# ksahlin/IsoCon

Hardware: AMD Instinct MI355X
Metric: read x candidate alignments/sec (NN-graph build, 50k x 2.5kb reads) (higher is better)
Workload: dtype u64; 1 GPU; C3: 50000 synthetic CCS reads (50000 unique), ~2500 bp, 10 isoforms, seed 30001; 1-set NN graph; edges=78526, graph_digest=65944c838d76a6c9, parallelism=single GPU

## Files before the change

### isocon_amd/csrc/isocon_hip.hip

```cpp
#include <algorithm>
#include <chrono>
#include <cstdio>
#include <cstdlib>
#include <cstring>
#include <numeric>
#include <string>
#include <memory>
#include <thread>
#include <vector>

#include "common.hpp"
#include "ed_band.hpp"
#include "ed_full.hpp"
#include "qgram_mm.hpp"
#include "nn.hpp"
#include "nn_list.hpp"
#include "nn_filter.hpp"
#include "nn_finalize.hpp"
#include "nn_finalize_host.hpp"
#include "partition_host.hpp"
#include "sg.hpp"
#include "msa.hpp"
#include "msa_build.hpp"
#include "msa_batch.hpp"
#include "hw.hpp"
#include "hw_tiles.hpp"
#include "ed_lanes.hpp"
#include "ed_bytes.hpp"

namespace isocon {
thread_local std::string g_last_error;
}

using namespace isocon;

static bool variant_lookup(const char *name, std::string *value)
{
    const char *e = getenv("ISOCON_DEBUG_VARIANT");
    if (!e) return false;
    const size_t ln = strlen(name);
    for (const char *p = e; *p;) {
        const char *q = strchr(p, ',');
        const size_t len = q ? (size_t)(q - p) : strlen(p);
        if (len >= ln && strncmp(p, name, ln) == 0 && (len == ln || p[ln] == '=')) {
            if (value) *value = len > ln ? std::string(p + ln + 1, len - ln - 1) : std::string();
            return true;
        }
        p += len + (q ? 1 : 0);
    }
    return false;
}
static bool variant(const char *name) { return variant_lookup(name, nullptr); }
static const char *variant_value(const char *name)
{
    thread_local std::string ring[8];
    thread_local unsigned at = 0;
    std::string &slot = ring[at++ % 8];
    return variant_lookup(name, &slot) ? slot.c_str() : nullptr;
}

struct BoundTag {
    bool valid = false, has_order = false;
    uint64_t serial = 0;
    QMap map = {0, 0, 0, 0};
    uint32_t depth = 0;
    int32_t kcap = 0;
    unsigned long long lb_total = 0;
};
struct MsaTag { bool valid = false; uint64_t serial = 0; uint32_t n_rows = 0, n_cols = 0; };
struct MsaBatchHost {
    bool valid = false;
    uint64_t serial = 0;
    uint32_t n_parts = 0, n_rows = 0;
    std::vector<uint32_t> ncols, col_base, first_row;
    std::vector<unsigned long long> m_off;
};
struct HeldHits { uint64_t store_serial = 0; uint64_t rows = 0; };

struct ScratchPool {
    struct Slot { void *p = nullptr; size_t cap = 0; };
    Slot slots[160];
    BoundTag bound_tag;
    HeldHits held_hits;
    MsaTag msa_tag;
    MsaBatchHost msab;
    void *get(int idx, size_t bytes)
    {
        Slot &s = slots[idx];
        if (bytes == 0) bytes = 16;
        if (s.cap < bytes) {
            if (s.p) (void)hipFree(s.p);
            s.p = nullptr; s.cap = 0;
            const size_t want = bytes + bytes / 8;
            if (hipMalloc(&s.p, want) == hipSuccess) s.cap = want;
            else if (hipMalloc(&s.p, bytes) == hipSuccess) s.cap = bytes;
            else { s.p = nullptr; (void)hipGetLastError(); }
        }
        return s.p;
    }
    void release()
    {
        for (Slot &s : slots) { if (s.p) (void)hipFree(s.p); s.p = nullptr; s.cap = 0; }
        bound_tag = BoundTag();
        held_hits = HeldHits();
        msa_tag = MsaTag();
        msab = MsaBatchHost();
    }
};

enum {
    SLOT_ED_TS = 0, SLOT_ED_IDS, SLOT_ED_K, SLOT_ED_OUT, SLOT_FULL_A, SLOT_FULL_B, SLOT_FULL_K, SLOT_FULL_OUT,
    SLOT_NN_BEST, SLOT_NN_QF, SLOT_NN_TF, SLOT_NN_HITS, SLOT_NN_HITCOUNT, SLOT_NN_STATS, SLOT_NN_TS, SLOT_NN_IDS, SLOT_NN_PLANES2, SLOT_NN_PERM, SLOT_NN_IL, SLOT_NN_IL2, SLOT_NN_HITS2, SLOT_NN_HITCOUNT2, SLOT_NN_QPROF, SLOT_NN_QSUM, SLOT_NN_LB, SLOT_NN_LBROW, SLOT_NN_LBLEN, SLOT_NN_SLOTORDER, SLOT_NN_LBCHUNKS, SLOT_NN_ROWMIN, SLOT_NN_COLMIN, SLOT_NN_SEED_A, SLOT_NN_SEED_B, SLOT_NN_SEED_N, SLOT_NN_LBT, SLOT_NN_LBT_OFF, SLOT_NN_LBT_SLO, SLOT_NN_LBT_LEN, SLOT_NN_LBT_PAD, SLOT_NN_SCORE, SLOT_NN_LDEST, SLOT_NN_FIN_HITS, SLOT_NN_FIN_CNT, SLOT_NN_FIN_START, SLOT_NN_FIN_CUR, SLOT_NN_FIN_NB, SLOT_NN_FIN_LEN2, SLOT_NN_FIN_ROWPTR, SLOT_NN_FIN_COLS, SLOT_NN_FIN_FLAG, SLOT_NN_FIN_BEST, SLOT_NN_ACC_HITS, SLOT_NN_LTOT, SLOT_NN_LCHUNKS, SLOT_NN_LIST, SLOT_NN_LPA, SLOT_NN_LPB, SLOT_NN_TEXT2, SLOT_NN_LTASKS,
    SLOT_SG_PAIRS, SLOT_SG_R, SLOT_SG_TRACE, SLOT_SG_END, SLOT_SG_OPS, SLOT_SG_CNT, SLOT_SG_RES, SLOT_SG_OFF, SLOT_SG_DENSE, SLOT_SG_BOUND, SLOT_SG_AOFF, SLOT_SG_ALNA, SLOT_SG_ALNB,
    SLOT_MSA_IN, SLOT_MSA_OUT, SLOT_MSA_DEG, SLOT_MSA_COUNTS, SLOT_MSA_MAJ, SLOT_MSA_FLAGS, SLOT_MSA_TOT, SLOT_MSA_NCAND, SLOT_MSA_LEN, SLOT_MSA_OFF, SLOT_MSA_PACKED, SLOT_MSA_ROWS, SLOT_MSA_OPS, SLOT_MSA_OPTR, SLOT_MSA_LONGEST, SLOT_MSA_WIDTH, SLOT_MSA_CSLOT, SLOT_MSA_LTOT, SLOT_MSA_WIDE, SLOT_MSA_PROW, SLOT_MSA_PCOL, SLOT_MSA_PPTR, SLOT_MSA_PBYTES, SLOT_MSAB_PART, SLOT_MSAB_FIRST, SLOT_MSAB_LM, SLOT_MSAB_SBASE, SLOT_MSAB_NCOLS, SLOT_MSAB_MOFF, SLOT_MSAB_CBASE, SLOT_MSAB_CBP, SLOT_MSAB_CBC, SLOT_MSAB_CBR,
    SLOT_HW_Q, SLOT_HW_T, SLOT_HW_K, SLOT_HW_OUT, SLOT_HW_TRACE, SLOT_HW_CTR, SLOT_HW_TILEQ, SLOT_HW_LANES, SLOT_HW_PQ, SLOT_HW_KEY, SLOT_HW_HIST, SLOT_HW_CURSOR, SLOT_HW_TBASE, SLOT_HW_CLS,
    SLOT_PACK_ASCII, SLOT_PACK_OFF, SLOT_PACK_BAD, SLOT_PACK_HIST, SLOT_PACK_FLAGS, SLOT_EB_A, SLOT_EB_B, SLOT_EB_K, SLOT_EB_OUT, SLOT_EB_ROWS, SLOT_SCAN_TMP, SLOT_SCAN_SUMS,
    SLOT_COUNT
};
static_assert(SLOT_COUNT <= 160, "ScratchPool::slots too small");

static ScratchPool g_scratch;

static uint64_t g_store_serial = 0;

struct isocon_store {
    uint64_t serial = ++g_store_serial;
    DevStore dev;
    explicit isocon_store(bool private_scratch = false) : own_pool(private_scratch ? new ScratchPool() : nullptr), pool(own_pool ? *own_pool : g_scratch) {}
    std::unique_ptr<ScratchPool> own_pool;
    ScratchPool &pool;
    std::vector<int32_t> lens;
    uint64_t device_bytes = 0;
    uint64_t *d_planes = nullptr;
    char alphabet[4] = {'A', 'C', 'G', 'T'};
    bool acgt = true;
    uint8_t *d_bytes = nullptr;
    uint64_t *d_boff = nullptr;
    uint64_t bytes_base = 0;
    std::vector<uint8_t> exc;
    std::vector<uint32_t> exc_count;
    uint32_t n_exc = 0;
    bool is_exc(uint32_t i) const { return n_exc != 0 && exc[i] != 0; }
    int32_t *d_lens = nullptr;
    int32_t maxlen = 0;
};

namespace {

struct PinnedStage {
    void *p = nullptr;
    size_t cap = 0;
    void *get(size_t bytes)
    {
        if (cap < bytes) {
            if (p) (void)hipHostFree(p);
            p = nullptr; cap = 0;
            if (hipHostMalloc(&p, bytes, hipHostMallocDefault) == hipSuccess) cap = bytes;
            else { p = nullptr; (void)hipGetLastError(); }
        }
        return p;
    }
    void release() { if (p) (void)hipHostFree(p); p = nullptr; cap = 0; }
};
static PinnedStage g_stage;
static constexpr size_t kStageBytes = (size_t)32 << 20;
static constexpr uint64_t kPackWaves = (uint64_t)1 << 25;
static constexpr size_t kStageMin = (size_t)32 << 10;

static std::vector<std::pair<const char *, size_t>> g_pinned;
static bool is_pinned(const void *p, size_t bytes)
{
    for (const auto &r : g_pinned)
        if ((const char *)p >= r.first && (const char *)p + bytes <= r.first + r.second) return true;
    return false;
}

static hipError_t copy_d2h(void *dst, const void *dsrc, size_t bytes)
{
    if (bytes < kStageMin || is_pinned(dst, bytes)) return hipMemcpy(dst, dsrc, bytes, hipMemcpyDeviceToHost);
    char *st = static_cast<char *>(g_stage.get(kStageBytes));
    if (!st) return hipMemcpy(dst, dsrc, bytes, hipMemcpyDeviceToHost);
    for (size_t off = 0; off < bytes; off += kStageBytes) {
        const size_t len = std::min(kStageBytes, bytes - off);
        const hipError_t e = hipMemcpy(st, static_cast<const char *>(dsrc) + off, len, hipMemcpyDeviceToHost);
        if (e != hipSuccess) return e;
        memcpy(static_cast<char *>(dst) + off, st, len);
    }
    return hipSuccess;
}

static hipError_t copy_h2d(void *ddst, const void *src, size_t bytes)
{
    if (bytes < kStageMin || is_pinned(src, bytes)) return hipMemcpy(ddst, src, bytes, hipMemcpyHostToDevice);
    char *st = static_cast<char *>(g_stage.get(kStageBytes));
    if (!st) return hipMemcpy(ddst, src, bytes, hipMemcpyHostToDevice);
    for (size_t off = 0; off < bytes; off += kStageBytes) {
        const size_t len = std::min(kStageBytes, bytes - off);
        memcpy(st, static_cast<const char *>(src) + off, len);
        const hipError_t e = hipMemcpy(static_cast<char *>(ddst) + off, st, len, hipMemcpyHostToDevice);
        if (e != hipSuccess) return e;
    }
    return hipSuccess;
}

struct DevBuf {
    void *p = nullptr;
    ScratchPool *pool = nullptr;
    int slot = -1;
    DevBuf() {}
    DevBuf(ScratchPool *pl, int sl) : pool(pl), slot(sl) {}
    DevBuf(const DevBuf &) = delete;
    DevBuf &operator=(const DevBuf &) = delete;
    ~DevBuf() { if (p && !pool) (void)hipFree(p); }
    template <class T> T *as() { return static_cast<T *>(p); }
    int alloc(size_t bytes)
    {
        if (pool) {
            p = pool->get(slot, bytes);
            if (!p) { g_last_error = "hipMalloc(scratch slot " + std::to_string(slot) + ", " + std::to_string(bytes) + " B) failed"; return ISOCON_E_HIP; }
            return ISOCON_OK;
        }
        if (p) { (void)hipFree(p); p = nullptr; }
        ISO_HIP_CHECK(hipMalloc(&p, bytes ? bytes : 16));
        return ISOCON_OK;
    }
};

template <int SHIFT, class OUT>
static int device_exscan(ScratchPool *pl, const uint32_t *d_in, uint32_t n, OUT *d_out)
{
    DevBuf d_tmp(pl, SLOT_SCAN_TMP), d_sums(pl, SLOT_SCAN_SUMS);
    const uint32_t tiles = std::max<uint32_t>(1, (n + SCAN_TILE - 1) / SCAN_TILE);
    int rc;
    if ((rc = d_tmp.alloc((size_t)std::max<uint32_t>(n, 1) * 4)) || (rc = d_sums.alloc((size_t)tiles * 8))) return rc;
    hipLaunchKernelGGL((k_scan_tiles<SHIFT>), dim3(tiles), dim3(256), 0, 0, d_in, n, d_tmp.as<uint32_t>(), d_sums.as<unsigned long long>());
    hipLaunchKernelGGL((k_scan_finish<OUT>), dim3(tiles), dim3(256), 0, 0, d_tmp.as<uint32_t>(), n, d_sums.as<unsigned long long>(), tiles, d_out, (unsigned long long *)nullptr);
    ISO_HIP_CHECK(hipGetLastError());
    return ISOCON_OK;
}

struct EventTimer {
    hipEvent_t e0 = nullptr, e1 = nullptr, em = nullptr;
    float total = 0.f;
    float marked_total = 0.f;
    bool marked = false;
    bool ok = false;
    EventTimer() { ok = hipEventCreate(&e0) == hipSuccess && hipEventCreate(&e1) == hipSuccess && hipEventCreate(&em) == hipSuccess; }
    ~EventTimer() { if (e0) (void)hipEventDestroy(e0); if (e1) (void)hipEventDestroy(e1); if (em) (void)hipEventDestroy(em); }
    void start() { if (ok) (void)hipEventRecord(e0, 0); marked = false; }
    void mark() { if (ok) { (void)hipEventRecord(em, 0); marked = true; } }
    float stop()
    {
        float ms = 0.f;
        if (ok) {
            (void)hipEventRecord(e1, 0); (void)hipEventSynchronize(e1); (void)hipEventElapsedTime(&ms, e0, e1);
            if (marked) { float part = 0.f; (void)hipEventElapsedTime(&part, em, e1); marked_total += part; marked = false; }
        }
        total += ms;
        return ms;
    }
};

struct PackMap { uint8_t sym[4]; };

__global__ __launch_bounds__(256) void k_byte_histogram(const uint8_t *__restrict__ ascii, uint64_t total, unsigned long long *__restrict__ hist)
{
    __shared__ uint32_t h[256];
    h[threadIdx.x] = 0;
    __syncthreads();
    for (uint64_t i = (uint64_t)blockIdx.x * 256 + threadIdx.x; i < total; i += (uint64_t)gridDim.x * 256) atomicAdd(&h[ascii[i]], 1u);
    __syncthreads();
    if (h[threadIdx.x]) atomicAdd(hist + threadIdx.x, (unsigned long long)h[threadIdx.x]);
}

__global__ __launch_bounds__(256) void k_pack_planes(const uint8_t *__restrict__ ascii, const uint64_t *__restrict__ offsets, uint64_t base, uint32_t n,
                                                      uint32_t nchunks, uint64_t *__restrict__ planes, unsigned long long *__restrict__ first_bad, PackMap map,
                                                      uint32_t fold, uint64_t w0)
{
    const uint64_t w = w0 + (uint64_t)blockIdx.x * 4 + (threadIdx.x >> 6);
    if (w >= (uint64_t)nchunks * n) return;
    const uint32_t lane = threadIdx.x & 63;
    const uint32_t chunk = (uint32_t)(w / n), seq = (uint32_t)(w % n);
    const uint64_t off = offsets[seq] - base, len = offsets[seq + 1] - offsets[seq];
    const uint64_t pos = (uint64_t)chunk * 64 + lane;
    int cd = 0;
    bool bad = false;
    if (pos < len) {
        uint8_t ch = ascii[off + pos];
        if (fold && ch >= 'a' && ch <= 'z') ch = (uint8_t)(ch - 32);
        cd = ch == map.sym[0] ? 0 : ch == map.sym[1] ? 1 : ch == map.sym[2] ? 2 : ch == map.sym[3] ? 3 : -1;
        bad = cd < 0 && !fold;
    }
    const unsigned long long lo = __ballot(!bad && (cd & 1)), hi = __ballot(!bad && (cd & 2)), bm = __ballot(bad);
    if (lane == 0) {
        planes[((size_t)chunk * n + seq) * 2] = lo;
        planes[((size_t)chunk * n + seq) * 2 + 1] = hi;
        if (bm) atomicMin(first_bad, ((unsigned long long)seq << 32) | ((unsigned long long)chunk * 64 + (unsigned long long)(__ffsll((long long)bm) - 1)));
    }
}

}

extern "C" {

const char *isocon_strerror(int status)
{
    switch (status) {
    case ISOCON_OK: return "ok";
    case ISOCON_E_ARG: return "bad argument";
    case ISOCON_E_ALPHABET: return "sequence contains a symbol outside ACGT";
    case ISOCON_E_HIP: return "HIP runtime error";
    case ISOCON_E_CAPACITY: return "output buffer too small";
    case ISOCON_E_NODEVICE: return "no usable GPU";
    case ISOCON_E_UNSUPPORTED: return "unsupported request";
    default: return "unknown status";
    }
}

const char *isocon_last_error(void) { return g_last_error.c_str(); }

int isocon_device_count(void)
{
    int n = 0;
    if (hipGetDeviceCount(&n) != hipSuccess) return 0;
    return n;
}

void isocon_release_scratch(void) { g_scratch.release(); g_stage.release(); }

int isocon_init(int device_ordinal)
{
    int n = 0;
    if (hipGetDeviceCount(&n) != hipSuccess || n <= 0) { g_last_error = "hipGetDeviceCount: no device"; return ISOCON_E_NODEVICE; }
    if (device_ordinal < 0 || device_ordinal >= n) return ISOCON_E_ARG;
    ISO_HIP_CHECK(hipSetDevice(device_ordinal));
    return ISOCON_OK;
}

static int store_create_impl(const uint8_t *ascii, const uint8_t *const *seq_ptrs, const uint64_t *offsets, uint32_t n, isocon_store **out, bool private_scratch = false)
{
    *out = nullptr;
    int32_t maxlen = 0;
    for (uint32_t i = 0; i < n; ++i) {
        if (offsets[i + 1] < offsets[i] || offsets[i + 1] - offsets[i] > 0x3fffffff) return ISOCON_E_ARG;
        maxlen = std::max<int32_t>(maxlen, (int32_t)(offsets[i + 1] - offsets[i]));
    }
    const uint32_t nchunks = (uint32_t)((maxlen + 63) / 64 + 1);
    const uint32_t nn = std::max<uint32_t>(n, 1);
    std::vector<int32_t> lens(nn, 0);
    for (uint32_t i = 0; i < n; ++i) lens[i] = (int32_t)(offsets[i + 1] - offsets[i]);
    const uint64_t base = n ? offsets[0] : 0, total = n ? offsets[n] - offsets[0] : 0;
    isocon_store *st = new isocon_store(private_scratch);
    st->lens = lens;
    st->maxlen = maxlen;
    const size_t pbytes = (size_t)nchunks * nn * 2 * sizeof(uint64_t), lbytes = lens.size() * sizeof(int32_t);
    if (hipMalloc((void **)&st->d_planes, pbytes) != hipSuccess || hipMalloc((void **)&st->d_lens, lbytes) != hipSuccess) {
        g_last_error = "hipMalloc(store) failed";
        isocon_store_destroy(st);
        return ISOCON_E_HIP;
    }
    {
        DevBuf d_ascii(&g_scratch, SLOT_PACK_ASCII), d_off(&g_scratch, SLOT_PACK_OFF), d_bad(&g_scratch, SLOT_PACK_BAD);
        uint64_t pack_waves = kPackWaves;
        if (const char *e = variant_value("pack_waves")) pack_waves = std::max<uint64_t>(4, strtoull(e, nullptr, 10)) & ~(uint64_t)3;
        const unsigned long long none = ~0ull;
        int rc = ISOCON_OK;
        if ((rc = d_ascii.alloc(total ? total : 16)) || (rc = d_off.alloc((size_t)(nn + 1) * 8)) || (rc = d_bad.alloc(8))) { isocon_store_destroy(st); return rc; }
        bool up = true;
        if (total && ascii) up = copy_h2d(d_ascii.p, ascii + base, total) == hipSuccess;
        else if (total) {
            char *stg = static_cast<char *>(g_stage.get(kStageBytes));
            hipEvent_t ev[2] = {nullptr, nullptr};
            up = stg != nullptr && hipEventCreateWithFlags(&ev[0], hipEventDisableTiming) == hipSuccess && hipEventCreateWithFlags(&ev[1], hipEventDisableTiming) == hipSuccess;
            const size_t half = kStageBytes / 2;
            uint64_t done = 0;
            bool busy[2] = {false, false};
            auto gather = [&](char *dst, uint64_t b0, uint64_t b1) {
                uint32_t i = (uint32_t)(std::upper_bound(offsets, offsets + n + 1, base + b0) - offsets) - 1;
                uint64_t in_seq = base + b0 - offsets[i];
                while (b0 < b1 && i < n) {
                    const uint64_t len = offsets[i + 1] - offsets[i];
                    const size_t take = (size_t)std::min<uint64_t>(len - in_seq, b1 - b0);
                    if (take) memcpy(dst, seq_ptrs[i] + in_seq, take);
                    dst += take; b0 += take; in_seq += take;
                    if (in_seq == len) { ++i; in_seq = 0; }
                }
            };
            const unsigned hc = std::thread::hardware_concurrency();
            const unsigned n_thr = total >= ((uint64_t)8 << 20) ? std::min(4u, hc ? hc : 1u) : 1u;
            for (int h = 0; up && done < total; h ^= 1) {
                if (busy[h]) up = hipEventSynchronize(ev[h]) == hipSuccess;
                const size_t fill = (size_t)std::min<uint64_t>(half, total - done);
                if (n_thr <= 1) gather(stg + h * half, done, done + fill);
                else {
                    std::thread th[4];
                    const size_t part = (fill + n_thr - 1) / n_thr;
                    for (unsigned t = 0; t < n_thr; ++t) {
                        const size_t a = std::min(fill, t * part), b = std::min(fill, (t + 1) * part);
                        th[t] = std::thread([&, a, b, h] { if (b > a) gather(stg + h * half + a, done + a, done + b); });
                    }
                    for (unsigned t = 0; t < n_thr; ++t) th[t].join();
                }
                up = up && hipMemcpyAsync(static_cast<char *>(d_ascii.p) + done, stg + h * half, fill, hipMemcpyHostToDevice, 0) == hipSuccess &&
                     hipEventRecord(ev[h], 0) == hipSuccess;
                busy[h] = true;
                done += fill;
            }
            up = up && hipStreamSynchronize(0) == hipSuccess;
            if (ev[0]) (void)hipEventDestroy(ev[0]);
            if (ev[1]) (void)hipEventDestroy(ev[1]);
        }
        bool ok = up &&
                  (n == 0 || copy_h2d(d_off.p, offsets, (size_t)(n + 1) * 8) == hipSuccess) &&
                  hipMemcpy(d_bad.p, &none, 8, hipMemcpyHostToDevice) == hipSuccess && copy_h2d(st->d_lens, lens.data(), lbytes) == hipSuccess;
        unsigned long long bad = none;
        if (ok) {
            if (n) {
                const uint64_t waves = (uint64_t)nchunks * n;
                for (uint64_t w0 = 0; w0 < waves; w0 += pack_waves)
                    hipLaunchKernelGGL(k_pack_planes, dim3((unsigned)((std::min<uint64_t>(pack_waves, waves - w0) + 3) / 4)), dim3(256), 0, 0, d_ascii.as<uint8_t>(), d_off.as<uint64_t>(), base, n, nchunks,
                                       st->d_planes, d_bad.as<unsigned long long>(), PackMap{{'A', 'C', 'G', 'T'}}, 0u, w0);
            } else {
                ok = hipMemset(st->d_planes, 0, pbytes) == hipSuccess;
            }
            ok = ok && hipGetLastError() == hipSuccess && hipMemcpy(&bad, d_bad.p, 8, hipMemcpyDeviceToHost) == hipSuccess;
        }
        if (!ok) {
            g_last_error = "isocon_store_create: device copy / packing failed";
            (void)hipGetLastError();
            isocon_store_destroy(st);
            return ISOCON_E_HIP;
        }
        if (bad != none) {
            DevBuf d_hist(&g_scratch, SLOT_PACK_HIST);
            unsigned long long hist[256];
            bool hok = d_hist.alloc(256 * 8) == ISOCON_OK && hipMemset(d_hist.p, 0, 256 * 8) == hipSuccess;
            if (hok) {
                hipLaunchKernelGGL(k_byte_histogram, dim3(1024), dim3(256), 0, 0, d_ascii.as<uint8_t>(), (uint64_t)total, d_hist.as<unsigned long long>());
                hok = hipGetLastError() == hipSuccess && hipMemcpy(hist, d_hist.p, sizeof(hist), hipMemcpyDeviceToHost) == hipSuccess;
            }
            int distinct = 0;
            for (int c = 0; hok && c < 256; ++c) distinct += hist[c] != 0;
            if (!hok) {
                g_last_error = "isocon_store_create: symbol histogram failed";
                (void)hipGetLastError();
                isocon_store_destroy(st);
                return ISOCON_E_HIP;
            }
            if (distinct > 4) {
                DevBuf d_flags(&g_scratch, SLOT_PACK_FLAGS);
                st->exc.assign(nn, 0);
                st->exc_count.assign(nn, 0);
                bool eok = d_flags.alloc((size_t)nn * 4) == ISOCON_OK && hipMemset(d_flags.p, 0, (size_t)nn * 4) == hipSuccess &&
                           hipMalloc((void **)&st->d_bytes, total ? total : 16) == hipSuccess && hipMalloc((void **)&st->d_boff, (size_t)(nn + 1) * 8) == hipSuccess;
                if (eok) {
                    const uint64_t waves = (uint64_t)nchunks * n;
                    for (uint64_t w0 = 0; w0 < waves; w0 += pack_waves)
                    hipLaunchKernelGGL(k_pack_planes, dim3((unsigned)((std::min<uint64_t>(pack_waves, waves - w0) + 3) / 4)), dim3(256), 0, 0, d_ascii.as<uint8_t>(), d_off.as<uint64_t>(), base, n, nchunks,
                                       st->d_planes, d_bad.as<unsigned long long>(), PackMap{{'A', 'C', 'G', 'T'}}, 1u, w0);
                    for (uint64_t w0 = 0; w0 < waves; w0 += pack_waves)
                        hipLaunchKernelGGL(k_exception_flags, dim3((unsigned)((std::min<uint64_t>(pack_waves, waves - w0) + 3) / 4)), dim3(256), 0, 0, d_ascii.as<uint8_t>(), d_off.as<uint64_t>(), base, n,
                                           nchunks, d_flags.as<uint32_t>(), (uint32_t)'A' | ((uint32_t)'C' << 8) | ((uint32_t)'G' << 16) | ((uint32_t)'T' << 24), w0);
                    eok = hipGetLastError() == hipSuccess && hipMemcpy(st->exc_count.data(), d_flags.p, (size_t)n * 4, hipMemcpyDeviceToHost) == hipSuccess &&
                          hipMemcpy(st->d_bytes, d_ascii.p, total, hipMemcpyDeviceToDevice) == hipSuccess &&
                          hipMemcpy(st->d_boff, d_off.p, (size_t)(n + 1) * 8, hipMemcpyDeviceToDevice) == hipSuccess;
                }
                if (!eok) {
                    g_last_error = "isocon_store_create: keeping the bytes of a set with more than four symbols failed";
                    (void)hipGetLastError();
                    isocon_store_destroy(st);
                    return ISOCON_E_HIP;
                }
                st->bytes_base = base;
                for (uint32_t i = 0; i < n; ++i) { st->exc[i] = st->exc_count[i] != 0; st->n_exc += st->exc[i]; }
                st->acgt = false;
                st->device_bytes += total + (size_t)(nn + 1) * 8;
            } else {
            PackMap map{{0, 0, 0, 0}};
            bool used[4] = {false, false, false, false};
            const char acgt_sym[4] = {'A', 'C', 'G', 'T'};
            for (int k = 0; k < 4; ++k) if (hist[(uint8_t)acgt_sym[k]]) { map.sym[k] = (uint8_t)acgt_sym[k]; used[k] = true; }
            for (int c = 0; c < 256; ++c) {
                if (!hist[c] || c == 'A' || c == 'C' || c == 'G' || c == 'T') continue;
                for (int k = 0; k < 4; ++k) if (!used[k]) { map.sym[k] = (uint8_t)c; used[k] = true; break; }
            }
            for (int k = 0; k < 4; ++k) if (!used[k]) { for (int c = 1; c < 256; ++c) if (!hist[c] && c != map.sym[0] && c != map.sym[1] && c != map.sym[2] && c != map.sym[3]) { map.sym[k] = (uint8_t)c; break; } }
            bool rok = hipMemcpy(d_bad.p, &none, 8, hipMemcpyHostToDevice) == hipSuccess;
            if (rok) {
                const uint64_t waves = (uint64_t)nchunks * n;
                for (uint64_t w0 = 0; w0 < waves; w0 += pack_waves)
                    hipLaunchKernelGGL(k_pack_planes, dim3((unsigned)((std::min<uint64_t>(pack_waves, waves - w0) + 3) / 4)), dim3(256), 0, 0, d_ascii.as<uint8_t>(), d_off.as<uint64_t>(), base, n, nchunks,
                                       st->d_planes, d_bad.as<unsigned long long>(), map, 0u, w0);
                rok = hipGetLastError() == hipSuccess && hipMemcpy(&bad, d_bad.p, 8, hipMemcpyDeviceToHost) == hipSuccess && bad == none;
            }
            if (!rok) {
                g_last_error = "isocon_store_create: packing under the set's own alphabet failed";
                (void)hipGetLastError();
                isocon_store_destroy(st);
                return ISOCON_E_HIP;
            }
            for (int k = 0; k < 4; ++k) st->alphabet[k] = (char)map.sym[k];
            st->acgt = false;
            }
        }
    }
    st->device_bytes += pbytes + lbytes;
    st->dev.planes = st->d_planes;
    st->dev.il = nullptr;
    st->dev.lens = st->d_lens;
    st->dev.n = n;
    st->dev.nchunks = nchunks;
    st->lens.resize(n);
    *out = st;
    return ISOCON_OK;
}

int isocon_store_create(const uint8_t *ascii, const uint64_t *offsets, uint32_t n, isocon_store **out)
{
    if (!out || (!ascii && n) || !offsets) return ISOCON_E_ARG;
    return store_create_impl(ascii, nullptr, offsets, n, out);
}

int isocon_store_create_ptrs(const uint8_t *const *seq_ptrs, const uint64_t *seq_lens, uint32_t n, isocon_store **out)
{
    if (!out || (n && (!seq_ptrs || !seq_lens))) return ISOCON_E_ARG;
    std::vector<uint64_t> offsets((size_t)n + 1, 0);
    for (uint32_t i = 0; i < n; ++i) {
        if (seq_lens[i] && !seq_ptrs[i]) return ISOCON_E_ARG;
        offsets[i + 1] = offsets[i] + seq_lens[i];
    }
    return store_create_impl(nullptr, seq_ptrs, offsets.data(), n, out);
}

int isocon_store_create_ptrs_ex(const uint8_t *const *seq_ptrs, const uint64_t *seq_lens, uint32_t n, uint32_t flags, isocon_store **out)
{
    if (!out || (n && (!seq_ptrs || !seq_lens)) || (flags & ~(uint32_t)ISOCON_STORE_PRIVATE_SCRATCH)) return ISOCON_E_ARG;
    std::vector<uint64_t> offsets((size_t)n + 1, 0);
    for (uint32_t i = 0; i < n; ++i) {
        if (seq_lens[i] && !seq_ptrs[i]) return ISOCON_E_ARG;
        offsets[i + 1] = offsets[i] + seq_lens[i];
    }
    return store_create_impl(nullptr, seq_ptrs, offsets.data(), n, out, (flags & ISOCON_STORE_PRIVATE_SCRATCH) != 0);
}

void *isocon_host_alloc(uint64_t bytes)
{
    void *p = nullptr;
    if (hipHostMalloc(&p, bytes ? bytes : 16, hipHostMallocDefault) != hipSuccess) { (void)hipGetLastError(); return nullptr; }
    g_pinned.emplace_back((const char *)p, (size_t)(bytes ? bytes : 16));
    return p;
}

void isocon_host_free(void *p)
{
    if (!p) return;
    for (size_t i = 0; i < g_pinned.size(); ++i)
        if (g_pinned[i].first == (const char *)p) { g_pinned.erase(g_pinned.begin() + (long)i); break; }
    (void)hipHostFree(p);
}

void isocon_store_destroy(isocon_store *s)
{
    if (!s) return;
    if (s->d_planes) (void)hipFree(s->d_planes);
    if (s->d_lens) (void)hipFree(s->d_lens);
    if (s->d_bytes) (void)hipFree(s->d_bytes);
    if (s->d_boff) (void)hipFree(s->d_boff);
    if (s->own_pool) s->own_pool->release();
    delete s;
}

uint32_t isocon_store_size(const isocon_store *s) { return s ? s->dev.n : 0; }
uint64_t isocon_store_device_bytes(const isocon_store *s) { return s ? s->device_bytes : 0; }

}

namespace {

template <int W>
int launch_band_tiles(isocon_store *st, const DevStore &S, const std::vector<uint32_t> &tile_shared, const std::vector<uint32_t> &lane_ids,
                      const std::vector<int32_t> &lane_k, std::vector<int32_t> &out, EventTimer &tm)
{
    const size_t nt = tile_shared.size();
    out.assign(nt * 64, -1);
    if (!nt) return ISOCON_OK;
    DevBuf d_ts(&st->pool, SLOT_ED_TS), d_ids(&st->pool, SLOT_ED_IDS), d_k(&st->pool, SLOT_ED_K), d_out(&st->pool, SLOT_ED_OUT);
    int rc;
    if ((rc = d_ts.alloc(nt * 4)) || (rc = d_ids.alloc(nt * 64 * 4)) || (rc = d_k.alloc(nt * 64 * 4)) || (rc = d_out.alloc(nt * 64 * 4))) return rc;
    ISO_HIP_CHECK(copy_h2d(d_ts.p, tile_shared.data(), nt * 4));
    ISO_HIP_CHECK(copy_h2d(d_ids.p, lane_ids.data(), nt * 64 * 4));
    ISO_HIP_CHECK(copy_h2d(d_k.p, lane_k.data(), nt * 64 * 4));
    tm.start();
    hipLaunchKernelGGL(k_ed_band_tiles<W>, dim3((unsigned)((nt + 3) / 4)), dim3(256), 0, 0, S, d_ts.as<uint32_t>(),
                       d_ids.as<uint32_t>(), d_k.as<int32_t>(), d_out.as<int32_t>(), (uint32_t)nt);
    ISO_HIP_CHECK(hipGetLastError());
    tm.stop();
    ISO_HIP_CHECK(copy_d2h(out.data(), d_out.p, nt * 64 * 4));
    return ISOCON_OK;
}

int run_band_stage(int W, isocon_store *st, const DevStore &S, const std::vector<uint32_t> &ts, const std::vector<uint32_t> &ids,
                   const std::vector<int32_t> &ks, std::vector<int32_t> &out, EventTimer &tm)
{
    switch (W) {
    case 1: return launch_band_tiles<1>(st, S, ts, ids, ks, out, tm);
    case 2: return launch_band_tiles<2>(st, S, ts, ids, ks, out, tm);
    case 4: return launch_band_tiles<4>(st, S, ts, ids, ks, out, tm);
    case 8: return launch_band_tiles<8>(st, S, ts, ids, ks, out, tm);
    default: return ISOCON_E_ARG;
    }
}

int run_full(isocon_store *st, const std::vector<uint32_t> &a, const std::vector<uint32_t> &b,
             const std::vector<int32_t> &k, std::vector<int32_t> &out, EventTimer &tm)
{
    const size_t np = a.size();
    out.assign(np, -1);
    if (!np) return ISOCON_OK;
    DevBuf d_a(&st->pool, SLOT_FULL_A), d_b(&st->pool, SLOT_FULL_B), d_k(&st->pool, SLOT_FULL_K), d_out(&st->pool, SLOT_FULL_OUT);
    int rc;
    if ((rc = d_a.alloc(np * 4)) || (rc = d_b.alloc(np * 4)) || (rc = d_k.alloc(np * 4)) || (rc = d_out.alloc(np * 4))) return rc;
    ISO_HIP_CHECK(copy_h2d(d_a.p, a.data(), np * 4));
    ISO_HIP_CHECK(copy_h2d(d_b.p, b.data(), np * 4));
    ISO_HIP_CHECK(copy_h2d(d_k.p, k.data(), np * 4));
    bool multipass = false;
    int32_t maxtext = 0;
    for (size_t p = 0; p < np; ++p) {
        const int32_t la = st->lens[a[p]], lb = st->lens[b[p]];
        if (std::min(la, lb) > 4096) multipass = true;
        maxtext = std::max(maxtext, std::max(la, lb));
    }
    const size_t lds = multipass ? (size_t)((maxtext + 15) & ~15) : 0;
    if (lds > 160 * 1024) { g_last_error = "sequence longer than 163840 bases in the un-banded kernel"; return ISOCON_E_UNSUPPORTED; }
    if (lds > 64 * 1024)
        ISO_HIP_CHECK(hipFuncSetAttribute((const void *)k_ed_full, hipFuncAttributeMaxDynamicSharedMemorySize, (int)lds));
    tm.start();
    hipLaunchKernelGGL(k_ed_full, dim3((unsigned)np), dim3(64), lds, 0, st->dev, d_a.as<uint32_t>(), d_b.as<uint32_t>(),
                       d_k.as<int32_t>(), d_out.as<int32_t>(), (uint32_t)np);
    ISO_HIP_CHECK(hipGetLastError());
    tm.stop();
    ISO_HIP_CHECK(copy_d2h(out.data(), d_out.p, np * 4));
    return ISOCON_OK;
}

int run_bytes(isocon_store *st, const std::vector<uint32_t> &a, const std::vector<uint32_t> &b, const std::vector<int32_t> &k, std::vector<int32_t> &out, EventTimer &tm)
{
    const size_t np = a.size();
    out.assign(np, -1);
    if (!np) return ISOCON_OK;
    if (!st->d_bytes) { g_last_error = "internal: byte-wise distances on a store that kept no bytes"; return ISOCON_E_HIP; }
    if (st->maxlen >= (int32_t)EB_INF - 1) { g_last_error = "byte-wise distances: sequences of 8 388 606 bases and more are not supported"; return ISOCON_E_UNSUPPORTED; }
    const uint32_t row_stride = (uint32_t)st->maxlen + 130u;
    size_t waves = std::min<size_t>(np, 8192);
    while (waves > 256 && waves * row_stride * 4 > ((size_t)2 << 30)) waves /= 2;
    DevBuf d_a(&st->pool, SLOT_EB_A), d_b(&st->pool, SLOT_EB_B), d_k(&st->pool, SLOT_EB_K), d_out(&st->pool, SLOT_EB_OUT), d_rows(&st->pool, SLOT_EB_ROWS);
    int rc;
    if ((rc = d_a.alloc(np * 4)) || (rc = d_b.alloc(np * 4)) || (rc = d_k.alloc(np * 4)) || (rc = d_out.alloc(np * 4)) || (rc = d_rows.alloc(waves * row_stride * 4))) return rc;
    ISO_HIP_CHECK(copy_h2d(d_a.p, a.data(), np * 4));
    ISO_HIP_CHECK(copy_h2d(d_b.p, b.data(), np * 4));
    ISO_HIP_CHECK(copy_h2d(d_k.p, k.data(), np * 4));
    tm.start();
    hipLaunchKernelGGL(k_ed_bytes, dim3((unsigned)waves), dim3(64), 0, 0, ByteStore{st->d_bytes, st->d_boff, st->bytes_base, st->d_lens}, d_a.as<uint32_t>(), d_b.as<uint32_t>(),
                       d_k.as<int32_t>(), (unsigned long long)np, d_rows.as<uint32_t>(), row_stride, d_out.as<int32_t>());
    ISO_HIP_CHECK(hipGetLastError());
    tm.stop();
    ISO_HIP_CHECK(copy_d2h(out.data(), d_out.p, np * 4));
    return ISOCON_OK;
}

}

namespace isocon {

int ed_pairs_impl(isocon_store *st, const uint32_t *a, const uint32_t *b, const int32_t *k, uint64_t n_pairs,
                  int32_t *out_ed, float *kernel_ms, uint64_t *full_pairs, bool images)
{
    EventTimer tm;
    const uint32_t n = st->dev.n;
    for (uint64_t p = 0; p < n_pairs; ++p)
        if (a[p] >= n || b[p] >= n) return ISOCON_E_ARG;
    bool swap_roles = false;
    {
        std::vector<uint8_t> seen_a(n, 0), seen_b(n, 0);
        size_t da = 0, db = 0;
        for (uint64_t p = 0; p < n_pairs; ++p) {
            if (!seen_a[a[p]]) { seen_a[a[p]] = 1; ++da; }
            if (!seen_b[b[p]]) { seen_b[b[p]] = 1; ++db; }
        }
        swap_roles = db < da;
    }
    std::vector<uint64_t> pending;
    pending.reserve(n_pairs);
    if (st->n_exc && !images) {
        std::vector<uint64_t> xp;
        for (uint64_t p = 0; p < n_pairs; ++p) (st->exc[a[p]] || st->exc[b[p]] ? xp : pending).push_back(p);
        if (!xp.empty()) {
            std::vector<uint32_t> xa(xp.size()), xb(xp.size());
            std::vector<int32_t> xk(xp.size()), res;
            for (size_t i = 0; i < xp.size(); ++i) { xa[i] = a[xp[i]]; xb[i] = b[xp[i]]; xk[i] = k ? k[xp[i]] : -1; }
            int rc = run_bytes(st, xa, xb, xk, res, tm);
            if (rc) return rc;
            for (size_t i = 0; i < xp.size(); ++i) out_ed[xp[i]] = res[i];
        }
    } else {
        pending.resize(n_pairs);
        std::iota(pending.begin(), pending.end(), 0);
    }
    static const int stages[4] = {1, 2, 4, 8};
    for (int si = 0; si < 4 && !pending.empty(); ++si) {
        const int W = stages[si];
        const int32_t kcap = 64 * W - 1;
        auto sh = [&](uint64_t p) { return swap_roles ? b[p] : a[p]; };
        auto ln = [&](uint64_t p) { return swap_roles ? a[p] : b[p]; };
        std::sort(pending.begin(), pending.end(), [&](uint64_t x, uint64_t y) {
            if (sh(x) != sh(y)) return sh(x) < sh(y);
            const int32_t lx = st->lens[ln(x)], ly = st->lens[ln(y)];
            if (lx != ly) return lx < ly;
            return x < y;
        });
        std::vector<uint64_t> todo = pending, next;
        if (W == 1) {
            const char *e = variant_value("ed_lanes");
            const size_t min_group = e ? (atoi(e) ? (size_t)-1 : 0) : 16;
            std::vector<uint64_t> lanes_p, tiles_p;
            for (size_t i = 0; i < todo.size();) {
                size_t j = i;
                while (j < todo.size() && sh(todo[j]) == sh(todo[i])) ++j;
                std::vector<uint64_t> &dst = (j - i) < min_group ? lanes_p : tiles_p;
                dst.insert(dst.end(), todo.begin() + i, todo.begin() + j);
                i = j;
            }
            if (!lanes_p.empty()) {
                const size_t np = lanes_p.size();
                std::vector<uint32_t> la(np), lb2(np);
                std::vector<int32_t> lk(np), res(np, -1);
                for (size_t i = 0; i < np; ++i) {
                    const uint64_t p = lanes_p[i];
                    la[i] = a[p]; lb2[i] = b[p];
                    const int32_t kr = k ? k[p] : -1;
                    lk[i] = kr < 0 ? kcap : std::min(kr, kcap);
                }
                DevBuf d_a(&st->pool, SLOT_ED_TS), d_b(&st->pool, SLOT_ED_IDS), d_k(&st->pool, SLOT_ED_K), d_out(&st->pool, SLOT_ED_OUT);
                int rc;
                if ((rc = d_a.alloc(np * 4)) || (rc = d_b.alloc(np * 4)) || (rc = d_k.alloc(np * 4)) || (rc = d_out.alloc(np * 4))) return rc;
                ISO_HIP_CHECK(copy_h2d(d_a.p, la.data(), np * 4));
                ISO_HIP_CHECK(copy_h2d(d_b.p, lb2.data(), np * 4));
                ISO_HIP_CHECK(copy_h2d(d_k.p, lk.data(), np * 4));
                NNParams none;
                memset(&none, 0, sizeof(none));
                tm.start();
                hipLaunchKernelGGL(k_ed_lanes<false>, dim3((unsigned)((np + 255) / 256)), dim3(256), 0, 0, st->dev, none, d_a.as<uint32_t>(), d_b.as<uint32_t>(),
                                   d_k.as<int32_t>(), (uint64_t)np, d_out.as<int32_t>());
                ISO_HIP_CHECK(hipGetLastError());
                tm.stop();
                ISO_HIP_CHECK(copy_d2h(res.data(), d_out.p, np * 4));
                for (size_t i = 0; i < np; ++i) {
                    const uint64_t p = lanes_p[i];
                    const int32_t kr = k ? k[p] : -1;
                    if (res[i] >= 0) out_ed[p] = res[i];
                    else if (kr >= 0 && kr <= kcap) out_ed[p] = -1;
                    else next.push_back(p);
                }
            }
            todo.swap(tiles_p);
        }
        for (int round = 0; round < 2 && !todo.empty(); ++round) {
            std::vector<uint32_t> ts, ids;
            std::vector<int32_t> ks;
            std::vector<uint64_t> slot_pair;
            size_t i = 0;
            while (i < todo.size()) {
                size_t j = i;
                const uint32_t s0 = sh(todo[i]);
                const size_t lim = round == 0 ? 64 : 1;
                while (j < todo.size() && j - i < lim && sh(todo[j]) == s0) ++j;
                ts.push_back(s0);
                for (size_t l = 0; l < 64; ++l) {
                    if (i + l < j) {
                        const uint64_t p = todo[i + l];
                        ids.push_back(ln(p));
                        const int32_t kr = k ? k[p] : -1;
                        ks.push_back(kr < 0 ? kcap : std::min(kr, kcap));
                        slot_pair.push_back(p);
                    } else {
                        ids.push_back(0xffffffffu);
                        ks.push_back(-1);
                        slot_pair.push_back(~(uint64_t)0);
                    }
                }
                i = j;
            }
            std::vector<int32_t> res;
            int rc = run_band_stage(W, st, st->dev, ts, ids, ks, res, tm);
            if (rc) return rc;
            std::vector<uint64_t> retry;
            for (size_t sidx = 0; sidx < slot_pair.size(); ++sidx) {
                const uint64_t p = slot_pair[sidx];
                if (p == ~(uint64_t)0) continue;
                const int32_t r = res[sidx];
                const int32_t kr = k ? k[p] : -1;
                if (r >= 0) out_ed[p] = r;
                else if (r == -2) retry.push_back(p);
                else if (kr >= 0 && kr <= kcap) out_ed[p] = -1;
                else next.push_back(p);
            }
            todo.swap(retry);
        }
        if (!todo.empty()) { g_last_error = "internal: single-lane tile undetermined"; return ISOCON_E_HIP; }
        pending.swap(next);
    }
    if (full_pairs) *full_pairs = pending.size();
    if (!pending.empty()) {
        std::vector<uint32_t> fa, fb;
        std::vector<int32_t> fk, res;
        for (uint64_t p : pending) { fa.push_back(a[p]); fb.push_back(b[p]); fk.push_back(k ? k[p] : -1); }
        int rc = run_full(st, fa, fb, fk, res, tm);
        if (rc) return rc;
        for (size_t i = 0; i < pending.size(); ++i) out_ed[pending[i]] = res[i];
    }
    if (kernel_ms) *kernel_ms = tm.total;
    return ISOCON_OK;
}

}

__global__ __launch_bounds__(256) void k_store_digest(const uint64_t *__restrict__ planes, size_t n_words, const int32_t *__restrict__ lens, uint32_t n,
                                                      unsigned long long *__restrict__ out)
{
    unsigned long long acc = 0;
    const size_t stride = (size_t)gridDim.x * blockDim.x;
    for (size_t i = (size_t)blockIdx.x * blockDim.x + threadIdx.x; i < n_words + n; i += stride) {
        unsigned long long v = i < n_words ? planes[i] : (unsigned long long)(uint32_t)lens[i - n_words];
        v ^= (unsigned long long)i * 0xD6E8FEB86659FD93ull;
        v ^= v >> 32; v *= 0x9E3779B97F4A7C15ull; v ^= v >> 29; v *= 0xBF58476D1CE4E5B9ull; v ^= v >> 32;
        acc += v;
    }
    for (int o = 32; o > 0; o >>= 1) acc += __shfl_xor(acc, o, 64);
    if ((threadIdx.x & 63) == 0 && acc) atomicAdd(out, acc);
}

extern "C" int isocon_store_digest(const isocon_store *s, uint64_t *out)
{
    if (!s || !out) return ISOCON_E_ARG;
    DevBuf d_acc;
    int rc;
    if ((rc = d_acc.alloc(8))) return rc;
    ISO_HIP_CHECK(hipMemset(d_acc.p, 0, 8));
    const size_t n_words = (size_t)s->dev.nchunks * std::max<uint32_t>(s->dev.n, 1) * 2;
    hipLaunchKernelGGL(k_store_digest, dim3(1024), dim3(256), 0, 0, s->d_planes, n_words, s->d_lens, s->dev.n, d_acc.as<unsigned long long>());
    ISO_HIP_CHECK(hipGetLastError());
    ISO_HIP_CHECK(hipMemcpy(out, d_acc.p, 8, hipMemcpyDeviceToHost));
    return ISOCON_OK;
}

extern "C" int isocon_ed_pairs(isocon_store *s, const uint32_t *a, const uint32_t *b, const int32_t *k, uint64_t n_pairs,
                               int32_t *out_ed, float *kernel_ms)
{
    if (!s || (n_pairs && (!a || !b || !out_ed))) return ISOCON_E_ARG;
    if (kernel_ms) *kernel_ms = 0.f;
    if (!n_pairs) return ISOCON_OK;
    return ed_pairs_impl(s, a, b, k, n_pairs, out_ed, kernel_ms, nullptr, false);
}

extern "C" int isocon_qgram_params(int32_t *out)
{
    if (out) { out[0] = QG_Q; out[1] = QG_B0; out[2] = QG_B1; out[3] = QG_CAP; }
    return QM_K;
}

namespace isocon {
int qgram_bounds_for_pairs(isocon_store *s, const uint32_t *a, const uint32_t *b, uint64_t n_pairs, int32_t *out_bound, float *kernel_ms)
{
    const uint32_t n = s->dev.n;
    const uint32_t n_pad = std::max<uint32_t>(QM_TILE, ((n + QM_TILE - 1) / QM_TILE) * QM_TILE);
    DevBuf d_prof(&s->pool, SLOT_NN_QPROF), d_sum(&s->pool, SLOT_NN_QSUM), d_a(&s->pool, SLOT_ED_TS), d_b(&s->pool, SLOT_ED_IDS), d_out(&s->pool, SLOT_ED_OUT);
    int rc;
    if ((rc = d_prof.alloc((size_t)n_pad * (QM_K / 2))) || (rc = d_sum.alloc((size_t)n * 4)) || (rc = d_a.alloc(n_pairs * 4)) || (rc = d_b.alloc(n_pairs * 4)) ||
        (rc = d_out.alloc(n_pairs * 4)))
        return rc;
    s->pool.bound_tag.valid = false;
    ISO_HIP_CHECK(copy_h2d(d_a.p, a, n_pairs * 4));
    ISO_HIP_CHECK(copy_h2d(d_b.p, b, n_pairs * 4));
    EventTimer tm;
    tm.start();
    hipLaunchKernelGGL(k_qgram_profile4, dim3((n + QP_SEQS - 1) / QP_SEQS), dim3(256), 0, 0, s->dev, d_prof.as<uint8_t>(), d_sum.as<uint32_t>(), n_pad);
    ISO_HIP_CHECK(hipGetLastError());
    for (uint64_t at = 0; at < n_pairs; at += (uint64_t)1 << 24) {
        const uint64_t cnt = std::min<uint64_t>((uint64_t)1 << 24, n_pairs - at);
        hipLaunchKernelGGL(k_qgram_lb_pairs, dim3((unsigned)((cnt + 3) / 4)), dim3(256), 0, 0, d_prof.as<uint8_t>(), d_sum.as<uint32_t>(), n_pad, d_a.as<uint32_t>() + at,
                           d_b.as<uint32_t>() + at, cnt, d_out.as<int32_t>() + at);
        ISO_HIP_CHECK(hipGetLastError());
    }
    const float ms = tm.stop();
    if (kernel_ms) *kernel_ms = ms;
    ISO_HIP_CHECK(copy_d2h(out_bound, d_out.p, n_pairs * 4));
    return ISOCON_OK;
}
}

extern "C" int isocon_qgram_bound_pairs(isocon_store *s, const uint32_t *a, const uint32_t *b, uint64_t n_pairs, int32_t *out_bound)
{
    if (!s || (n_pairs && (!a || !b || !out_bound))) return ISOCON_E_ARG;
    if (!n_pairs) return ISOCON_OK;
    if (s->n_exc) { g_last_error = "q-gram bounds are defined on the 2-bit planes: the set holds more than four distinct symbols"; return ISOCON_E_ALPHABET; }
    const uint32_t n = s->dev.n;
    for (uint64_t i = 0; i < n_pairs; ++i)
        if (a[i] >= n || b[i] >= n) { g_last_error = "pair index out of range"; return ISOCON_E_ARG; }
    return qgram_bounds_for_pairs(s, a, b, n_pairs, out_bound, nullptr);
}

extern "C" int isocon_block_bound_pairs(isocon_store *s, const uint32_t *owner, const uint32_t *partner, uint64_t n_pairs, int32_t probe_stride, int32_t *out_count)
{
    if (probe_stride != 4 && probe_stride != 2) return ISOCON_E_ARG;
    if (!s || (n_pairs && (!owner || !partner || !out_count))) return ISOCON_E_ARG;
    if (!n_pairs) return ISOCON_OK;
    if (s->n_exc) { g_last_error = "block bounds are defined on the 2-bit planes: the set holds more than four distinct symbols"; return ISOCON_E_ALPHABET; }
    const uint32_t n = s->dev.n;
    if (n_pairs >= ((uint64_t)1 << 31)) return ISOCON_E_ARG;
    for (uint64_t i = 0; i < n_pairs; ++i)
        if (owner[i] >= n || partner[i] >= n) { g_last_error = "pair index out of range"; return ISOCON_E_ARG; }
    const uint32_t stride = nnf_text2_stride(s->maxlen);
    DevBuf d_text(&s->pool, SLOT_NN_TEXT2), d_a(&s->pool, SLOT_ED_TS), d_b(&s->pool, SLOT_ED_IDS), d_out(&s->pool, SLOT_ED_OUT);
    int rc;
    if ((rc = d_text.alloc((size_t)n * stride * 4)) || (rc = d_a.alloc(n_pairs * 4)) || (rc = d_b.alloc(n_pairs * 4)) || (rc = d_out.alloc(n_pairs * 4))) return rc;
    ISO_HIP_CHECK(copy_h2d(d_a.p, owner, n_pairs * 4));
    ISO_HIP_CHECK(copy_h2d(d_b.p, partner, n_pairs * 4));
    hipLaunchKernelGGL(k_build_text2, dim3(n), dim3(256), 0, 0, s->dev, d_text.as<uint32_t>(), stride);
    hipLaunchKernelGGL(k_nn_block_count_pairs, dim3((unsigned)n_pairs), dim3(256), 0, 0, d_text.as<uint32_t>(), stride, s->dev.lens, d_a.as<uint32_t>(), d_b.as<uint32_t>(), d_out.as<int32_t>(), probe_stride);
    ISO_HIP_CHECK(hipGetLastError());
    ISO_HIP_CHECK(copy_d2h(out_count, d_out.p, n_pairs * 4));
    return ISOCON_OK;
}

#include "nn_context.inc"
#include "nn_bounds.inc"
#include "nn_lists.inc"
#include "nn_main.inc"
#include "nn_wide.inc"
#include "nn_images.inc"
#include "nn_entry.inc"
#include "sg_host.inc"
#include "msa_host.inc"
#include "hw_host.inc"

extern "C" int isocon_partition_ids(uint32_t n, const int32_t *degree, uint64_t n_edges, const uint32_t *edge_a, const uint32_t *edge_b,
                                    const uint32_t *rank, int32_t nbr_tiebreak, uint32_t *out_centre, int64_t *out_weight,
                                    uint64_t *out_member_ptr, uint32_t *out_members, uint32_t *n_parts)
{
    if (!out_member_ptr || !n_parts || (n && (!degree || !rank || !out_centre || !out_weight || !out_members)) || (n_edges && (!edge_a || !edge_b))) return ISOCON_E_ARG;
    return partition_ids_impl(n, degree, n_edges, edge_a, edge_b, rank, nbr_tiebreak, out_centre, out_weight, out_member_ptr, out_members, n_parts);
}
```

### isocon_amd/csrc/nn_bounds.inc

```

namespace {

int NNContext::build_bounds(const QMap &Q, int32_t kcap, NNParams &P, bool want_seeds)
{
    const uint32_t q_begin = Q.begin, q_end = Q.end;
    P.lb = nullptr;
    P.lb_row = nullptr;
    P.slot_order = nullptr;
    if (variant("nn_no_qgram") || n < 2 || n >= (1u << 30) || q_begin >= q_end) return ISOCON_OK;
    if (!want_seeds && st->pool.bound_tag.valid && st->pool.bound_tag.serial == st->serial && st->pool.bound_tag.map.same(Q) &&
        st->pool.bound_tag.depth == depth && st->pool.bound_tag.kcap == kcap) {
        P.lb = static_cast<const uint8_t *>(st->pool.slots[SLOT_NN_LB].p);
        P.lb_row = static_cast<const unsigned long long *>(st->pool.slots[SLOT_NN_LBROW].p);
        if (st->pool.bound_tag.has_order && use_slot_order(Q.count())) P.slot_order = static_cast<const uint32_t *>(st->pool.slots[SLOT_NN_SLOTORDER].p);
        lb_total = st->pool.bound_tag.lb_total;
        return ISOCON_OK;
    }
    st->pool.bound_tag.valid = false;
    const uint32_t nq = Q.count();
    const std::vector<int32_t> &lens = st->lens;
    const uint32_t n_pad = std::max<uint32_t>(QM_TILE, ((n + QM_TILE - 1) / QM_TILE) * QM_TILE);
    const size_t prof_bytes = (size_t)n_pad * (QM_K / 2);
    d_qprof.pool = d_qsum.pool = &st->pool;
    d_qprof.slot = SLOT_NN_QPROF; d_qsum.slot = SLOT_NN_QSUM;
    HostClock bclk;
    {
        size_t free_b = 0, total_b = 0;
        if (hipMemGetInfo(&free_b, &total_b) != hipSuccess || prof_bytes > free_b / 2 + st->pool.slots[SLOT_NN_QPROF].cap) return ISOCON_OK;
        if (d_qprof.alloc(prof_bytes) || d_qsum.alloc((size_t)n * 4)) return ISOCON_OK;
    }
    bclk.lap("bounds: memory check + profile buffers");
    tm.start();
    hipLaunchKernelGGL(k_qgram_profile4, dim3((n + QP_SEQS - 1) / QP_SEQS), dim3(256), 0, 0, st->dev, d_qprof.as<uint8_t>(), d_qsum.as<uint32_t>(), n_pad);
    ISO_HIP_CHECK(hipGetLastError());
    struct StopTimer { NNContext &c; bool armed = true; ~StopTimer() { if (armed) c.stats.bound_kernel_ms += c.tm.stop(); } } stop_timer{*this};
    std::vector<unsigned long long> &off = lb_off_host;
    std::vector<uint32_t> &rlen = lb_len_host;
    off.assign(nq, 0);
    rlen.assign(nq, 0);
    unsigned long long total = 0, sum_rlen = 0;
    uint64_t hi = 0;
    const uint32_t nrb = (nq + QM_TILE - 1) / QM_TILE;
    std::vector<uint64_t> rb_lo(nrb, ~(uint64_t)0), rb_hi(nrb, 0);
    for (uint32_t s = 0; s < nq; ++s) {
        const uint64_t q = Q.entry(s);
        if (hi < q + 1) hi = q + 1;
        while (hi < n && lens[hi] - lens[q] <= kcap) ++hi;
        uint64_t len = hi - q - 1;
        if (len > depth) len = depth;
        const uint64_t pal = (q + 1) & ~(uint64_t)15;
        off[s] = total + (q + 1 - pal);
        rlen[s] = (uint32_t)len;
        sum_rlen += len;
        if (len) {
            total += ((q + 1 + len + 15) & ~(uint64_t)15) - pal;
            rb_lo[s / QM_TILE] = std::min<uint64_t>(rb_lo[s / QM_TILE], q + 1);
            rb_hi[s / QM_TILE] = std::max<uint64_t>(rb_hi[s / QM_TILE], q + len);
        }
    }
    if (total == 0) return ISOCON_OK;
    bclk.lap("bounds: profile launch + rows (host)");
    const unsigned long long totalT = sum_rlen + 30ull * n;
    bclk.lap("bounds: transposed rows (host)");
    size_t free_b = 0, total_b = 0;
    const size_t need = (size_t)total + (size_t)totalT + prof_bytes + (size_t)n * 24 + (size_t)nq * 12;
    if (hipMemGetInfo(&free_b, &total_b) != hipSuccess || need > free_b / 2 + st->pool.slots[SLOT_NN_LB].cap + st->pool.slots[SLOT_NN_QPROF].cap) return ISOCON_OK;
    bclk.lap("bounds: memory check 2");
    std::vector<uint2> tiles;
    for (uint32_t g = 0; g * 4 < nrb; ++g) {
        uint64_t jmin = ~(uint64_t)0, jmax = 0;
        bool any = false;
        for (uint32_t I = g * 4; I < std::min(nrb, g * 4 + 4); ++I)
            if (rb_lo[I] != ~(uint64_t)0) { any = true; jmin = std::min(jmin, rb_lo[I] / QM_TILE); jmax = std::max(jmax, rb_hi[I] / QM_TILE); }
        if (!any) continue;
        for (uint64_t j0 = jmin; j0 <= jmax; j0 += 8)
            for (uint32_t ri = 0; ri < 4; ++ri)
                for (uint32_t cj = 0; cj < 8; ++cj) {
                    const uint32_t I = g * 4 + ri;
                    const uint64_t J = j0 + cj;
                    const bool have = I < nrb && rb_lo[I] != ~(uint64_t)0 && J >= rb_lo[I] / QM_TILE && J <= rb_hi[I] / QM_TILE;
                    tiles.push_back(have ? make_uint2(I, (uint32_t)J) : make_uint2(0xffffffffu, 0xffffffffu));
                }
    }
    while (tiles.size() % 256) tiles.push_back(make_uint2(0xffffffffu, 0xffffffffu));
    if (tiles.size() > 0x7fffffffull) return ISOCON_OK;
    bclk.lap("bounds: tile table (host)");
    d_lb.pool = d_lbrow.pool = d_lblen.pool = &st->pool;
    d_lb.slot = SLOT_NN_LB; d_lbrow.slot = SLOT_NN_LBROW; d_lblen.slot = SLOT_NN_LBLEN;
    int rc;
    if ((rc = d_lb.alloc((size_t)total)) ||
        (rc = d_lbrow.alloc((size_t)nq * 8)) || (rc = d_lblen.alloc((size_t)nq * 4)))
        return ISOCON_OK;
    d_lbt.pool = d_offT.pool = d_sloT.pool = d_lenT.pool = d_score.pool = &st->pool;
    d_lbt.slot = SLOT_NN_LBT; d_offT.slot = SLOT_NN_LBT_OFF; d_sloT.slot = SLOT_NN_LBT_SLO; d_lenT.slot = SLOT_NN_LBT_LEN; d_score.slot = SLOT_NN_SCORE;
    DevBuf d_padT(&st->pool, SLOT_NN_LBT_PAD);
    if (d_lbt.alloc((size_t)totalT + 16) || d_offT.alloc(((size_t)n + 1) * 8) || d_sloT.alloc((size_t)n * 4) || d_lenT.alloc((size_t)n * 4) || d_score.alloc((size_t)n * 4) ||
        d_padT.alloc((size_t)n * 4))
        return ISOCON_OK;
    ISO_HIP_CHECK(hipMemsetAsync(d_score.p, 0, (size_t)n * 4, 0));
    d_chunks.pool = &st->pool;
    d_chunks.slot = SLOT_NN_LBCHUNKS;
    if (d_chunks.alloc(tiles.size() * sizeof(uint2))) return ISOCON_OK;
    ISO_HIP_CHECK(copy_h2d(d_chunks.p, tiles.data(), tiles.size() * sizeof(uint2)));
    ISO_HIP_CHECK(copy_h2d(d_lbrow.p, off.data(), (size_t)nq * 8));
    ISO_HIP_CHECK(copy_h2d(d_lblen.p, rlen.data(), (size_t)nq * 4));
    hipLaunchKernelGGL(k_lbt_rows, dim3((n + 255) / 256), dim3(256), 0, 0, Q, nq, d_lblen.as<uint32_t>(), n, d_sloT.as<uint32_t>(), d_lenT.as<uint32_t>(), d_padT.as<uint32_t>());
    if ((rc = device_exscan<0, unsigned long long>(&st->pool, d_padT.as<uint32_t>(), n, d_offT.as<unsigned long long>()))) return ISOCON_OK;
    hipLaunchKernelGGL(k_lbt_offsets, dim3((n + 255) / 256), dim3(256), 0, 0, n, d_sloT.as<uint32_t>(), d_offT.as<unsigned long long>());
    ISO_HIP_CHECK(hipGetLastError());
    bclk.lap("bounds: alloc + uploads");
    if (use_slot_order(nq)) {
        std::vector<uint32_t> order(nq);
        std::iota(order.begin(), order.end(), 0u);
        std::stable_sort(order.begin(), order.end(), [&](uint32_t x, uint32_t y) { return rlen[x] > rlen[y]; });
        d_order.pool = &st->pool;
        d_order.slot = SLOT_NN_SLOTORDER;
        if (d_order.alloc((size_t)nq * 4)) return ISOCON_OK;
        ISO_HIP_CHECK(copy_h2d(d_order.p, order.data(), (size_t)nq * 4));
    }
    unsigned long long *rowmin = nullptr, *colmin = nullptr;
    if (want_seeds) {
        d_rowmin.pool = d_colmin.pool = d_seed_a.pool = d_seed_b.pool = &st->pool;
        d_rowmin.slot = SLOT_NN_ROWMIN; d_colmin.slot = SLOT_NN_COLMIN; d_seed_a.slot = SLOT_NN_SEED_A; d_seed_b.slot = SLOT_NN_SEED_B;
        if (!(d_rowmin.alloc((size_t)nq * 8 * QM_SEEDS) || d_colmin.alloc((size_t)n_pad * 8 * QM_SEEDS) || d_seed_a.alloc((size_t)n * 8 * QM_SEEDS) || d_seed_b.alloc((size_t)n * 8 * QM_SEEDS))) {
            ISO_HIP_CHECK(hipMemsetAsync(d_rowmin.p, 0xff, (size_t)nq * 8 * QM_SEEDS, 0));
            ISO_HIP_CHECK(hipMemsetAsync(d_colmin.p, 0xff, (size_t)n_pad * 8 * QM_SEEDS, 0));
            rowmin = d_rowmin.as<unsigned long long>();
            colmin = d_colmin.as<unsigned long long>();
        }
    }
    bclk.lap("bounds: slot order + seed buffers");
    static bool lds_attr_set = false;
    if (!lds_attr_set) {
        ISO_HIP_CHECK(hipFuncSetAttribute((const void *)k_qgram_mm, hipFuncAttributeMaxDynamicSharedMemorySize, (int)QM_LDS_BYTES));
        lds_attr_set = true;
    }
    tm.mark();
    hipLaunchKernelGGL(k_qgram_mm, dim3((unsigned)tiles.size()), dim3(512), QM_LDS_BYTES, 0, d_qprof.as<uint8_t>(), d_qsum.as<uint32_t>(), n, n_pad,
                       d_chunks.as<uint2>(), d_lbrow.as<unsigned long long>(), d_lblen.as<uint32_t>(), d_lb.as<uint8_t>(), Q, nq,
                       d_qf.as<uint8_t>(), d_tf.as<uint8_t>(), rowmin, colmin, d_offT.as<unsigned long long>(), d_sloT.as<uint32_t>(), d_lenT.as<uint32_t>(),
                       d_lbt.as<uint8_t>(), d_score.as<uint32_t>());
    ISO_HIP_CHECK(hipGetLastError());
    stop_timer.armed = false;
    {
        const float before = tm.marked_total;
        stats.bound_kernel_ms += tm.stop();
        stats.mm_kernel_ms += tm.marked_total - before;
        tm.marked_total = before;
    }
    bclk.lap("bounds: k_qgram_mm (wait)");
#ifdef ISOCON_QM_TIMELINE
    {
        const size_t nt = std::min<size_t>(tiles.size(), 16384);
        std::vector<unsigned long long> tl(nt * 8);
        ISO_HIP_CHECK(hipMemcpyFromSymbol(tl.data(), HIP_SYMBOL(g_qm_timeline), nt * 64));
        double sum[5] = {0, 0, 0, 0, 0};
        unsigned long long t_min = ~0ull, t_max = 0;
        size_t cnt = 0;
        for (size_t b = 0; b < nt; ++b) {
            if (tiles[b].x == 0xffffffffu) continue;
            const unsigned long long *t = tl.data() + b * 8;
            for (int k = 0; k < 5; ++k) sum[k] += (double)(t[k + 1] - t[k]);
            t_min = std::min(t_min, t[0]); t_max = std::max(t_max, t[5]);
            ++cnt;
        }
        fprintf(stderr, "[qm timeline] %zu tiles: prologue %.2f us, K loop %.2f us, E1 %.2f us, E2 %.2f us, E3 %.2f us per tile; first start to last end %.3f ms\n", cnt,
                sum[0] / cnt / 100.0, sum[1] / cnt / 100.0, sum[2] / cnt / 100.0, sum[3] / cnt / 100.0, sum[4] / cnt / 100.0, (double)(t_max - t_min) / 1e5);
    }
#endif
    for (const uint2 &t : tiles) stats.bound_tiles += t.x != 0xffffffffu;
    P.lb = d_lb.as<uint8_t>();
    P.lb_row = d_lbrow.as<unsigned long long>();
    if (use_slot_order(nq)) P.slot_order = d_order.as<uint32_t>();
    seeds_ready = rowmin != nullptr;
    seed_nq = nq;
    lb_total = total;
    st->pool.bound_tag.valid = true;
    st->pool.bound_tag.lb_total = total;
    st->pool.bound_tag.has_order = use_slot_order(nq);
    st->pool.bound_tag.serial = st->serial;
    st->pool.bound_tag.map = Q; st->pool.bound_tag.depth = depth; st->pool.bound_tag.kcap = kcap;
    return ISOCON_OK;
}

int NNContext::run_bound_seeds(const QMap &Q)
{
    if (!seeds_ready) return ISOCON_OK;
    tm.start();
    const uint64_t np = (uint64_t)2 * QM_SEEDS * n;
    const uint32_t ranks = std::max<uint32_t>(1u, Q.stride >> Q.block_log2);
    uint32_t col_classes = QM_SEEDS;
    while (col_classes > 1 && col_classes * ranks > (uint32_t)QM_SEEDS) col_classes >>= 1;
    if (const char *e = variant_value("nn_seed_classes")) { const int v = atoi(e); if (v == 1 || v == 2 || v == QM_SEEDS) col_classes = (uint32_t)v; }
    DevBuf d_seed_n(&st->pool, SLOT_NN_SEED_N);
    int rc;
    if ((rc = d_seed_n.alloc(8))) return rc;
    ISO_HIP_CHECK(hipMemsetAsync(d_seed_n.p, 0, 8, 0));
    ISO_HIP_CHECK(hipMemsetAsync(d_seed_a.p, 0xff, (size_t)np * 4, 0));
    ISO_HIP_CHECK(hipMemsetAsync(d_seed_b.p, 0xff, (size_t)np * 4, 0));
    hipLaunchKernelGGL(k_qgram_seed_pairs, dim3((n + 255) / 256), dim3(256), 0, 0, d_rowmin.as<unsigned long long>(), d_colmin.as<unsigned long long>(),
                       n, Q, seed_nq, col_classes, d_seed_a.as<uint32_t>(), d_seed_b.as<uint32_t>(), d_seed_n.as<unsigned long long>());
    ISO_HIP_CHECK(hipGetLastError());
    hipLaunchKernelGGL(k_ed_lanes<true>, dim3((unsigned)((np + 255) / 256)), dim3(256), 0, 0, st->dev, params(63), d_seed_a.as<uint32_t>(), d_seed_b.as<uint32_t>(),
                       (const int32_t *)nullptr, np, (int32_t *)nullptr);
    ISO_HIP_CHECK(hipGetLastError());
    stats.seed_kernel_ms += tm.stop();
    return ISOCON_OK;
}

}
```

### isocon_amd/csrc/nn_context.inc

```

namespace {

struct HostClock {
    std::chrono::steady_clock::time_point t0 = std::chrono::steady_clock::now();
    const bool on = getenv("ISOCON_DEBUG") != nullptr;
    void lap(const char *what)
    {
        if (!on) return;
        const auto t1 = std::chrono::steady_clock::now();
        fprintf(stderr, "[isocon] %-28s %8.2f ms\n", what, std::chrono::duration<double, std::milli>(t1 - t0).count());
        t0 = t1;
    }
};

struct NNContext {
    isocon_store *st = nullptr;
    uint32_t n = 0;
    std::vector<uint8_t> qflag, tflag;
    bool two_set = false;
    std::vector<uint8_t> wide_mask;
    int32_t min_d = 1;
    uint32_t depth = 0x7fffffffu;
    DevBuf d_best, d_qf, d_tf, d_hits, d_hit_count, d_stats;
    DevBuf d_text;
    uint32_t text_stride = 0;
    bool text_ready = false;
    DevBuf d_qprof, d_qsum, d_lb, d_lbrow, d_lblen;
    DevBuf d_chunks;
    DevBuf d_lbt, d_offT, d_sloT, d_lenT, d_score;
    DevBuf d_order;
    DevBuf d_rowmin, d_colmin, d_seed_a, d_seed_b;
    uint64_t hits_cap = 0;
    std::vector<int32_t> best;
    std::vector<int32_t> hits;
    isocon_nn_stats stats;
    EventTimer tm;

    bool ensure_text()
    {
        if (text_ready) return true;
        text_stride = (uint32_t)NN_TEXT_PAD_FRONT + (uint32_t)((st->maxlen + 7) / 8) + (uint32_t)NN_TEXT_PAD_BACK;
        size_t free_b = 0, total_b = 0;
        if (hipMemGetInfo(&free_b, &total_b) != hipSuccess || (size_t)n * text_stride * 4 > free_b / 2) return false;
        d_text.pool = &st->pool;
        d_text.slot = SLOT_NN_IL;
        if (d_text.alloc((size_t)std::max<uint32_t>(n, 1) * text_stride * 4) != ISOCON_OK) return false;
        hipLaunchKernelGGL(k_build_nibble_text, dim3(std::max<uint32_t>(n, 1)), dim3(256), 0, 0, st->dev, d_text.as<uint32_t>(), text_stride);
        if (hipGetLastError() != hipSuccess) return false;
        text_ready = true;
        return true;
    }
    DevBuf d_text2;
    uint32_t text2_stride = 0;
    bool text2_ready = false;
    bool ensure_text2()
    {
        if (text2_ready) return true;
        text2_stride = nnf_text2_stride(st->maxlen);
        size_t free_b = 0, total_b = 0;
        if (hipMemGetInfo(&free_b, &total_b) != hipSuccess || (size_t)n * text2_stride * 4 > free_b / 2 + st->pool.slots[SLOT_NN_TEXT2].cap) return false;
        d_text2.pool = &st->pool;
        d_text2.slot = SLOT_NN_TEXT2;
        if (d_text2.alloc((size_t)std::max<uint32_t>(n, 1) * text2_stride * 4) != ISOCON_OK) return false;
        hipLaunchKernelGGL(k_build_text2, dim3(std::max<uint32_t>(n, 1)), dim3(256), 0, 0, st->dev, d_text2.as<uint32_t>(), text2_stride);
        if (hipGetLastError() != hipSuccess) return false;
        text2_ready = true;
        return true;
    }
    static bool use_slot_order(uint32_t nq)
    {
        if (const char *e = variant_value("nn_order")) return atoi(e) != 0;
        return nq <= 16384;
    }
    int build_bounds(const QMap &Q, int32_t kcap, NNParams &P, bool want_seeds = false);
    std::vector<unsigned long long> lb_off_host;
    std::vector<uint32_t> lb_len_host;
    unsigned long long lb_total = 0;
    bool seeds_ready = false;
    uint32_t seed_nq = 0;
    int run_bound_seeds(const QMap &Q);
    DevBuf d_ltot, d_lchunks, d_list, d_lpa, d_lpb, d_lmeta, d_ltasks;
    struct ListPlan {
        bool listed = false;
        unsigned long long n_chunks = 0, n_chunks_narrow = 0, n_small = 0;
        unsigned long long conv_a = 0, conv_b = 0, conv_pairs = 0;
        NNChunk *a = nullptr, *b = nullptr, *sorted_a = nullptr, *sorted_b = nullptr;
    };
    int plan_lists(const QMap &Q, uint32_t nq, const NNParams &PR, ListPlan &L);
    NNParams params(int32_t kcap)
    {
        NNParams P;
        P.best = d_best.as<int32_t>();
        P.qflag = d_qf.as<uint8_t>();
        P.tflag = d_tf.as<uint8_t>();
        P.hits = d_hits.as<int32_t>();
        P.hit_count = d_hit_count.as<unsigned long long>();
        P.stats = d_stats.as<unsigned long long>();
        P.hits_cap = hits_cap;
        P.kcap = kcap;
        P.min_d = image_pass ? 0 : min_d;
        P.depth = depth;
        P.fixed = fixed ? 1 : 0;
        P.q_list = nullptr;
        P.own = QMap{0u, n, 1u, 0u};
        P.lb = nullptr;
        P.lb_row = nullptr;
        P.slot_order = nullptr;
        P.wg_base = 0;
        P.chunks = nullptr;
        P.list = nullptr;
        return P;
    }

    int upload_best() { ISO_HIP_CHECK(copy_h2d(d_best.p, best.data(), (size_t)n * 4)); return ISOCON_OK; }
    int download_best() { ISO_HIP_CHECK(copy_d2h(best.data(), d_best.p, (size_t)n * 4)); return ISOCON_OK; }
    int reset_counters()
    {
        ISO_HIP_CHECK(hipMemset(d_hit_count.p, 0, 8));
        ISO_HIP_CHECK(hipMemset(d_stats.p, 0, 2 * (NN_COUNTER_SLOTS * 4 + 1) * 8));
        return ISOCON_OK;
    }
    bool keep_dev = false;
    const int32_t *dev_hits = nullptr;
    uint64_t dev_hit_count = 0;
    int collect(std::vector<int32_t> &out, uint64_t *needed, bool filter = false, bool to_device = false)
    {
        unsigned long long cnt = 0;
        ISO_HIP_CHECK(hipMemcpy(&cnt, d_hit_count.p, 8, hipMemcpyDeviceToHost));
        unsigned long long sc2[2][NN_COUNTER_SLOTS * 4 + 1];
        ISO_HIP_CHECK(hipMemcpy(sc2, d_stats.p, sizeof(sc2), hipMemcpyDeviceToHost));
        for (int blk = 0; blk < 2; ++blk) {
            const unsigned long long *sc = sc2[blk];
            stats.pairs_prefiltered += sc[NN_COUNTER_SLOTS * 4];
            for (int i = 0; i < NN_COUNTER_SLOTS; ++i) {
                stats.pairs_evaluated += sc[i * 4 + 0];
                stats.cells_columns += sc[i * 4 + 1];
                stats.tiles += sc[i * 4 + 2];
                stats.live_columns += sc[i * 4 + 3];
                if (blk == 1) stats.narrow_columns += sc[i * 4 + 1];
            }
        }
        if (needed) *needed = cnt;
        if (cnt > hits_cap) return ISOCON_E_CAPACITY;
        stats.hits += cnt;
        const void *src = d_hits.p;
        if (filter && cnt > 4096 && dev_hit_count == 0) {
            DevBuf d_h2(&st->pool, SLOT_NN_HITS2), d_c2(&st->pool, SLOT_NN_HITCOUNT2);
            int rc;
            if ((rc = d_h2.alloc((size_t)cnt * 12)) || (rc = d_c2.alloc(8))) return rc;
            ISO_HIP_CHECK(hipMemset(d_c2.p, 0, 8));
            const unsigned blocks = (unsigned)std::min<unsigned long long>((cnt + 255) / 256, 4096);
            hipLaunchKernelGGL(k_filter_hits, dim3(blocks), dim3(256), 0, 0, d_hits.as<int32_t>(), cnt, d_best.as<int32_t>(), d_h2.as<int32_t>(),
                               d_c2.as<unsigned long long>());
            ISO_HIP_CHECK(hipGetLastError());
            ISO_HIP_CHECK(hipMemcpy(&cnt, d_c2.p, 8, hipMemcpyDeviceToHost));
            src = d_h2.p;
        }
        if (to_device) {
            dev_hits = static_cast<const int32_t *>(src);
            dev_hit_count = cnt;
            return ISOCON_OK;
        }
        const size_t base = out.size();
        out.resize(base + (size_t)cnt * 3);
        if (cnt) ISO_HIP_CHECK(copy_d2h(out.data() + base, src, (size_t)cnt * 12));
        return ISOCON_OK;
    }
    int pull_dev_hits()
    {
        if (dev_hit_count) {
            const size_t base = hits.size();
            hits.resize(base + (size_t)dev_hit_count * 3);
            ISO_HIP_CHECK(copy_d2h(hits.data() + base, dev_hits, (size_t)dev_hit_count * 12));
        }
        dev_hits = nullptr;
        dev_hit_count = 0;
        return ISOCON_OK;
    }
    bool is_exc(uint32_t q) const { return st->n_exc != 0 && st->exc[q] != 0; }
    bool mask_exc = true;
    bool image_pass = false;
    bool fixed = false;
    bool dev_excluded(uint32_t q) const { return mask_exc && is_exc(q); }
    bool flags_dirty = false;
    int upload_flags()
    {
        if (!n) return ISOCON_OK;
        if (!st->n_exc || !mask_exc) {
            ISO_HIP_CHECK(copy_h2d(d_qf.p, qflag.data(), n));
            ISO_HIP_CHECK(copy_h2d(d_tf.p, tflag.data(), n));
            return ISOCON_OK;
        }
        std::vector<uint8_t> q2(qflag), t2(tflag);
        for (uint32_t i = 0; i < n; ++i)
            if (st->exc[i]) q2[i] = t2[i] = 0;
        ISO_HIP_CHECK(copy_h2d(d_qf.p, q2.data(), n));
        ISO_HIP_CHECK(copy_h2d(d_tf.p, t2.data(), n));
        return ISOCON_OK;
    }
    bool admissible(uint32_t x, uint32_t y) const { return qflag[x] && tflag[y]; }
    void apply(uint32_t s, uint32_t p, int32_t d)
    {
        if (d < min_d) return;
        const int32_t ls = st->lens[s], lp = st->lens[p];
        if (admissible(s, p) && d <= ls && d <= best[s]) { if (!fixed) best[s] = d; hits.push_back((int32_t)s); hits.push_back((int32_t)p); hits.push_back(d); }
        if (admissible(p, s) && d <= lp && d <= best[p]) { if (!fixed) best[p] = d; hits.push_back((int32_t)p); hits.push_back((int32_t)s); hits.push_back(d); }
    }
};

template <int W>
int launch_nn_tiles(NNContext &C, const std::vector<uint32_t> &ts, const std::vector<uint32_t> &ids, int32_t kcap, float *ms_out)
{
    const size_t nt = ts.size();
    if (!nt) return ISOCON_OK;
    DevBuf d_ts(&C.st->pool, SLOT_NN_TS), d_ids(&C.st->pool, SLOT_NN_IDS);
    int rc;
    if ((rc = d_ts.alloc(nt * 4)) || (rc = d_ids.alloc(nt * 64 * 4))) return rc;
    ISO_HIP_CHECK(copy_h2d(d_ts.p, ts.data(), nt * 4));
    ISO_HIP_CHECK(copy_h2d(d_ids.p, ids.data(), nt * 64 * 4));
    C.tm.start();
    hipLaunchKernelGGL(k_nn_tiles<W>, dim3((unsigned)((nt + 3) / 4)), dim3(256), 0, 0, C.st->dev, C.params(kcap),
                       d_ts.as<uint32_t>(), d_ids.as<uint32_t>(), (uint32_t)nt);
    ISO_HIP_CHECK(hipGetLastError());
    const float ms = C.tm.stop();
    if (ms_out) *ms_out += ms;
    return ISOCON_OK;
}

int run_nn_tiles(int W, NNContext &C, const std::vector<uint32_t> &ts, const std::vector<uint32_t> &ids, float *ms_out)
{
    switch (W) {
    case 1: return launch_nn_tiles<1>(C, ts, ids, 63, ms_out);
    case 2: return launch_nn_tiles<2>(C, ts, ids, 127, ms_out);
    case 4: return launch_nn_tiles<4>(C, ts, ids, 255, ms_out);
    case 8: return launch_nn_tiles<8>(C, ts, ids, 511, ms_out);
    default: return ISOCON_E_ARG;
    }
}

void push_tiles(std::vector<uint32_t> &ts, std::vector<uint32_t> &ids, uint32_t shared, const std::vector<uint32_t> &lanes)
{
    for (size_t i = 0; i < lanes.size(); i += 64) {
        ts.push_back(shared);
        for (size_t l = 0; l < 64; ++l) ids.push_back(i + l < lanes.size() ? lanes[i + l] : 0xffffffffu);
    }
}

void length_window(const std::vector<int32_t> &lens, uint32_t x, int32_t w, uint32_t &lo, uint32_t &hi)
{
    const int32_t L = lens[x];
    lo = (uint32_t)(std::lower_bound(lens.begin(), lens.end(), L - w) - lens.begin());
    hi = (uint32_t)(std::upper_bound(lens.begin(), lens.end(), L + w) - lens.begin());
}

int nn_setup(NNContext &C, isocon_store *s, const uint8_t *is_converged, const uint8_t *is_target, uint64_t depth,
             const int32_t *best_in)
{
    C.st = s;
    C.n = s->dev.n;
    C.d_best.pool = C.d_qf.pool = C.d_tf.pool = C.d_hits.pool = C.d_hit_count.pool = C.d_stats.pool = &s->pool;
    C.d_best.slot = SLOT_NN_BEST; C.d_qf.slot = SLOT_NN_QF; C.d_tf.slot = SLOT_NN_TF; C.d_hits.slot = SLOT_NN_HITS;
    C.d_hit_count.slot = SLOT_NN_HITCOUNT; C.d_stats.slot = SLOT_NN_STATS;
    const uint32_t n = C.n;
    for (uint32_t i = 1; i < n; ++i)
        if (s->lens[i] < s->lens[i - 1]) { g_last_error = "nearest-neighbour entry points need a length-sorted store"; return ISOCON_E_ARG; }
    C.two_set = is_target != nullptr;
    C.min_d = C.two_set ? 0 : 1;
    C.qflag.assign(n, 0);
    C.tflag.assign(n, 0);
    uint64_t n_targets = 0;
    for (uint32_t i = 0; i < n; ++i) {
        if (C.two_set) { C.tflag[i] = is_target[i] ? 1 : 0; C.qflag[i] = is_target[i] ? 0 : 1; n_targets += C.tflag[i]; }
        else { C.tflag[i] = 1; C.qflag[i] = (is_converged && is_converged[i]) ? 0 : 1; }
    }
    if (C.two_set) {
        if (depth < n_targets) { g_last_error = "2-set search with neighbor_search_depth < number of targets is not supported"; return ISOCON_E_UNSUPPORTED; }
        C.depth = 0x7fffffffu;
    } else {
        if (depth == 0) { g_last_error = "neighbor_search_depth must be >= 1"; return ISOCON_E_ARG; }
        C.depth = depth > 0x7fffffffull ? 0x7fffffffu : (uint32_t)depth;
    }
    HostClock clk;
    C.best.assign(std::max<uint32_t>(n, 1), NN_INF);
    if (best_in) std::copy(best_in, best_in + n, C.best.begin());
    clk.lap("setup: host arrays");
    memset(&C.stats, 0, sizeof(C.stats));
    C.hits_cap = ((uint64_t)1 << 20) + (uint64_t)n * 48;
    if (const char *e = variant_value("hits_cap")) C.hits_cap = std::max<uint64_t>(16, strtoull(e, nullptr, 10));
    int rc;
    if ((rc = C.d_best.alloc((size_t)std::max<uint32_t>(n, 1) * 4)) || (rc = C.d_qf.alloc(std::max<uint32_t>(n, 1))) ||
        (rc = C.d_tf.alloc(std::max<uint32_t>(n, 1))) || (rc = C.d_hits.alloc(C.hits_cap * 12)) || (rc = C.d_hit_count.alloc(8)) ||
        (rc = C.d_stats.alloc(2 * (NN_COUNTER_SLOTS * 4 + 1) * 8)))
        return rc;
    clk.lap("setup: pool");
    if ((rc = C.upload_flags())) return rc;
    clk.lap("setup: role flags");
    return ISOCON_OK;
}

bool qmap_args_ok(uint32_t q_stride, uint32_t q_block) { return q_stride != 0 && q_block != 0 && (q_block & (q_block - 1)) == 0 && q_block <= q_stride; }
QMap qmap_of(uint32_t q_begin, uint32_t q_end, uint32_t q_stride, uint32_t q_block)
{
    uint32_t lg = 0;
    while ((1u << lg) < q_block) ++lg;
    return QMap{q_begin, q_end, q_stride, lg};
}

}
```

### isocon_amd/csrc/nn_entry.inc

```

namespace {

int nn_phase_a(NNContext &C, const QMap &Q, bool allow_regroup = false, bool do_seed = true, bool do_main = true, bool seeded_before = false)
{
    if (!C.st->n_exc || !do_main) return nn_phase_a_planes(C, Q, allow_regroup, do_seed, do_main, seeded_before);
    return nn_phase_a_images(C, Q, allow_regroup, do_seed, seeded_before);
}

int nn_phase_b(NNContext &C, const QMap &Q)
{
    return C.st->n_exc ? nn_phase_b_images(C, Q) : nn_phase_b_planes(C, Q);
}


int nn_finalize_device_core(ScratchPool *pl, uint32_t n, const int32_t *d_best, const int32_t *best_host, const int32_t *d_hits, uint64_t n_hits,
                            int32_t *out_best, uint64_t *out_row_ptr, uint32_t *out_cols, uint64_t cols_cap, uint64_t *n_cols_needed)
{
    DevBuf d_cnt(pl, SLOT_NN_FIN_CNT), d_start(pl, SLOT_NN_FIN_START), d_cur(pl, SLOT_NN_FIN_CUR), d_nb(pl, SLOT_NN_FIN_NB),
        d_len2(pl, SLOT_NN_FIN_LEN2), d_rowptr(pl, SLOT_NN_FIN_ROWPTR), d_cols(pl, SLOT_NN_FIN_COLS), d_flag(pl, SLOT_NN_FIN_FLAG);
    int rc;
    if ((rc = d_cnt.alloc((size_t)n * 4)) || (rc = d_start.alloc(((size_t)n + 1) * 8)) || (rc = d_cur.alloc((size_t)n * 4)) ||
        (rc = d_nb.alloc((size_t)n_hits * 4 + 16)) || (rc = d_len2.alloc((size_t)n * 4)) || (rc = d_rowptr.alloc(((size_t)n + 1) * 8)) ||
        (rc = d_cols.alloc((size_t)n_hits * 4 + 16)) || (rc = d_flag.alloc(4)))
        return rc;
    ISO_HIP_CHECK(hipMemsetAsync(d_cnt.p, 0, (size_t)n * 4, 0));
    ISO_HIP_CHECK(hipMemsetAsync(d_cur.p, 0, (size_t)n * 4, 0));
    ISO_HIP_CHECK(hipMemsetAsync(d_flag.p, 0, 4, 0));
    const unsigned hb = (unsigned)std::max<uint64_t>(1, (n_hits + 255) / 256), nb_ = (n + 255) / 256;
    hipLaunchKernelGGL(k_fin_count, dim3(hb), dim3(256), 0, 0, d_hits, (unsigned long long)n_hits, d_best, n, d_cnt.as<uint32_t>());
    if ((rc = device_exscan<0, unsigned long long>(pl, d_cnt.as<uint32_t>(), n, d_start.as<unsigned long long>()))) return rc;
    hipLaunchKernelGGL(k_fin_scatter, dim3(hb), dim3(256), 0, 0, d_hits, (unsigned long long)n_hits, d_best, n,
                       d_start.as<unsigned long long>(), d_cur.as<uint32_t>(), d_nb.as<uint32_t>());
    hipLaunchKernelGGL(k_fin_rows, dim3(nb_), dim3(256), 0, 0, n, d_start.as<unsigned long long>(), d_nb.as<uint32_t>(), d_len2.as<uint32_t>(), d_flag.as<uint32_t>());
    if ((rc = device_exscan<0, unsigned long long>(pl, d_len2.as<uint32_t>(), n, d_rowptr.as<unsigned long long>()))) return rc;
    hipLaunchKernelGGL(k_fin_gather, dim3(nb_), dim3(256), 0, 0, n, d_start.as<unsigned long long>(), d_nb.as<uint32_t>(), d_rowptr.as<unsigned long long>(), d_cols.as<uint32_t>());
    ISO_HIP_CHECK(hipGetLastError());
    uint32_t flag = 0;
    ISO_HIP_CHECK(hipMemcpy(&flag, d_flag.p, 4, hipMemcpyDeviceToHost));
    if (flag) return ISOCON_E_UNSUPPORTED;
    static_assert(sizeof(unsigned long long) == sizeof(uint64_t), "row pointers travel as they are");
    ISO_HIP_CHECK(copy_d2h(out_row_ptr, d_rowptr.p, ((size_t)n + 1) * 8));
    const uint64_t total = out_row_ptr[n];
    if (n_cols_needed) *n_cols_needed = total;
    if (total > cols_cap) return ISOCON_E_CAPACITY;
    if (total) ISO_HIP_CHECK(copy_d2h(out_cols, d_cols.p, (size_t)total * 4));
    for (uint32_t i = 0; i < n; ++i) out_best[i] = out_row_ptr[i + 1] > out_row_ptr[i] ? best_host[i] : -1;
    return ISOCON_OK;
}

int nn_finalize_device(isocon_store *st, uint32_t n, const int32_t *best, const int32_t *hits, uint64_t n_hits, int32_t *out_best,
                       uint64_t *out_row_ptr, uint32_t *out_cols, uint64_t cols_cap, uint64_t *n_cols_needed)
{
    ScratchPool *pl = &st->pool;
    DevBuf d_hits(pl, SLOT_NN_FIN_HITS), d_best(pl, SLOT_NN_FIN_BEST);
    int rc;
    if ((rc = d_hits.alloc((size_t)n_hits * 12)) || (rc = d_best.alloc((size_t)n * 4))) return rc;
    ISO_HIP_CHECK(copy_h2d(d_hits.p, hits, (size_t)n_hits * 12));
    ISO_HIP_CHECK(copy_h2d(d_best.p, best, (size_t)n * 4));
    return nn_finalize_device_core(pl, n, d_best.as<int32_t>(), best, d_hits.as<int32_t>(), n_hits, out_best, out_row_ptr, out_cols, cols_cap, n_cols_needed);
}


}

extern "C" int isocon_nn_partial(isocon_store *s, const uint8_t *is_converged, const uint8_t *is_target, uint64_t depth,
                                 uint32_t q_begin, uint32_t q_end, uint32_t q_stride, uint32_t q_block, int32_t phase, int32_t *best_inout,
                                 int32_t *out_hits, uint64_t hits_cap, uint64_t *n_hits, isocon_nn_stats *stats, const uint8_t *wide_queries)
{
    if (!s || !best_inout || !n_hits || (hits_cap && !out_hits) || phase < 0 || phase > 3 || !qmap_args_ok(q_stride, q_block)) return ISOCON_E_ARG;
    const uint32_t n = s->dev.n;
    if (q_end > n) q_end = n;
    const QMap Q = qmap_of(q_begin, q_end, q_stride, q_block);
    NNContext C;
    int rc = nn_setup(C, s, is_converged, is_target, depth, best_inout);
    if (rc) return rc;
    if (phase == 2 && wide_queries) C.wide_mask.assign(wide_queries, wide_queries + n);
    rc = phase == 2 ? nn_phase_b(C, Q) : nn_phase_a(C, Q, false, phase == 0 || phase == 3, phase == 1 || phase == 3, phase == 1);
    if (rc) return rc;
    C.stats.kernel_ms = C.tm.total; C.stats.narrow_kernel_ms = C.tm.marked_total;
    if (stats) *stats = C.stats;
    std::copy(C.best.begin(), C.best.begin() + n, best_inout);
    *n_hits = C.hits.size() / 3;
    if (*n_hits > hits_cap) return ISOCON_E_CAPACITY;
    if (!C.hits.empty()) memcpy(out_hits, C.hits.data(), C.hits.size() * 4);
    return ISOCON_OK;
}

extern "C" int isocon_nn_finalize(uint32_t n, const int32_t *best, const int32_t *hits, uint64_t n_hits,
                                  int32_t *out_best, uint64_t *out_row_ptr, uint32_t *out_cols, uint64_t cols_cap,
                                  uint64_t *n_cols_needed)
{
    if ((n && (!best || !out_best)) || !out_row_ptr || (n_hits && !hits) || (cols_cap && !out_cols)) return ISOCON_E_ARG;
    return nn_finalize_impl(n, best, hits, n_hits, out_best, out_row_ptr, out_cols, cols_cap, n_cols_needed);
}

extern "C" int isocon_nn_partial_dev(isocon_store *s, const uint8_t *is_converged, const uint8_t *is_target, uint64_t depth,
                                     uint32_t q_begin, uint32_t q_end, uint32_t q_stride, uint32_t q_block, int32_t phase, int32_t *best_inout_dev,
                                     int32_t keep_hits, uint64_t *n_hits_held, isocon_nn_stats *stats, const uint8_t *wide_queries)
{
    if (!s || !best_inout_dev || !n_hits_held || phase < 0 || phase > 3 || !qmap_args_ok(q_stride, q_block)) return ISOCON_E_ARG;
    const uint32_t n = s->dev.n;
    if (q_end > n) q_end = n;
    const QMap Q = qmap_of(q_begin, q_end, q_stride, q_block);
    std::vector<int32_t> best(std::max<uint32_t>(n, 1), NN_INF);
    if (n) ISO_HIP_CHECK(copy_d2h(best.data(), best_inout_dev, (size_t)n * 4));
    NNContext C;
    int rc = nn_setup(C, s, is_converged, is_target, depth, best.data());
    if (rc) return rc;
    if (phase == 2 && wide_queries) C.wide_mask.assign(wide_queries, wide_queries + n);
    C.keep_dev = phase != 2;
    rc = phase == 2 ? nn_phase_b(C, Q) : nn_phase_a(C, Q, false, phase == 0 || phase == 3, phase == 1 || phase == 3, phase == 1);
    if (rc) return rc;
    C.stats.kernel_ms = C.tm.total; C.stats.narrow_kernel_ms = C.tm.marked_total;
    if (stats) *stats = C.stats;
    if (n) ISO_HIP_CHECK(copy_h2d(best_inout_dev, C.best.data(), (size_t)n * 4));
    if (!keep_hits || s->pool.held_hits.store_serial != s->serial) s->pool.held_hits = HeldHits{s->serial, 0};
    const uint64_t add_host = C.hits.size() / 3, add = add_host + C.dev_hit_count, have = s->pool.held_hits.rows;
    ScratchPool::Slot &slot = s->pool.slots[SLOT_NN_ACC_HITS];
    if ((have + add) * 12 > slot.cap) {
        void *bigger = nullptr;
        const size_t want = (size_t)(have + add) * 12 * 2 + ((size_t)1 << 20);
        ISO_HIP_CHECK(hipMalloc(&bigger, want));
        if (have) ISO_HIP_CHECK(hipMemcpy(bigger, slot.p, (size_t)have * 12, hipMemcpyDeviceToDevice));
        if (slot.p) (void)hipFree(slot.p);
        slot.p = bigger; slot.cap = want;
    }
    if (add_host) ISO_HIP_CHECK(copy_h2d(static_cast<char *>(slot.p) + (size_t)have * 12, C.hits.data(), (size_t)add_host * 12));
    if (C.dev_hit_count)
        ISO_HIP_CHECK(hipMemcpy(static_cast<char *>(slot.p) + (size_t)(have + add_host) * 12, C.dev_hits, (size_t)C.dev_hit_count * 12, hipMemcpyDeviceToDevice));
    s->pool.held_hits.rows = have + add;
    *n_hits_held = s->pool.held_hits.rows;
    return ISOCON_OK;
}

extern "C" int isocon_nn_hits_dev(isocon_store *s, const int32_t *best_dev, int32_t *out_hits_dev, uint64_t cap_rows, uint64_t *n_kept)
{
    if (!s || !best_dev || (cap_rows && !out_hits_dev)) return ISOCON_E_ARG;
    uint64_t rows = s->pool.held_hits.store_serial == s->serial ? s->pool.held_hits.rows : 0;
    if (s->pool.slots[SLOT_NN_ACC_HITS].cap < rows * 12) rows = 0;
    if (rows > cap_rows) return ISOCON_E_CAPACITY;
    if (cap_rows) ISO_HIP_CHECK(hipMemsetAsync(out_hits_dev, 0xff, (size_t)cap_rows * 12, 0));
    unsigned long long kept = 0;
    if (rows) {
        DevBuf d_c(&s->pool, SLOT_NN_HITCOUNT2);
        int rc;
        if ((rc = d_c.alloc(8))) return rc;
        ISO_HIP_CHECK(hipMemsetAsync(d_c.p, 0, 8, 0));
        const unsigned blocks = (unsigned)std::min<unsigned long long>((rows + 255) / 256, 4096);
        hipLaunchKernelGGL(k_filter_hits, dim3(blocks), dim3(256), 0, 0, static_cast<const int32_t *>(s->pool.slots[SLOT_NN_ACC_HITS].p), (unsigned long long)rows,
                           best_dev, out_hits_dev, d_c.as<unsigned long long>());
        ISO_HIP_CHECK(hipGetLastError());
        if (n_kept) ISO_HIP_CHECK(hipMemcpy(&kept, d_c.p, 8, hipMemcpyDeviceToHost));
    }
    if (n_kept) *n_kept = kept;
    return ISOCON_OK;
}

extern "C" int isocon_nn_finalize_dev(isocon_store *s, const int32_t *best_dev, const int32_t *hits_dev, uint64_t n_rows,
                                      int32_t *out_best, uint64_t *out_row_ptr, uint32_t *out_cols, uint64_t cols_cap, uint64_t *n_cols_needed)
{
    if (!s || !out_row_ptr || (n_rows && !hits_dev) || (cols_cap && !out_cols)) return ISOCON_E_ARG;
    const uint32_t n = s->dev.n;
    if (n && (!best_dev || !out_best)) return ISOCON_E_ARG;
    std::vector<int32_t> best(std::max<uint32_t>(n, 1));
    if (n) ISO_HIP_CHECK(copy_d2h(best.data(), best_dev, (size_t)n * 4));
    int rc = nn_finalize_device_core(&s->pool, n, best_dev, best.data(), hits_dev, n_rows, out_best, out_row_ptr, out_cols, cols_cap, n_cols_needed);
    if (rc != ISOCON_E_UNSUPPORTED) return rc;
    std::vector<int32_t> hits((size_t)n_rows * 3);
    if (n_rows) ISO_HIP_CHECK(copy_d2h(hits.data(), hits_dev, (size_t)n_rows * 12));
    return nn_finalize_impl(n, best.data(), hits.data(), n_rows, out_best, out_row_ptr, out_cols, cols_cap, n_cols_needed);
}

extern "C" int isocon_nn_graph(isocon_store *s, const uint8_t *is_converged, const uint8_t *is_target, uint64_t depth,
                               int32_t *out_best, uint64_t *out_row_ptr, uint32_t *out_cols, uint64_t cols_cap,
                               uint64_t *n_cols_needed, isocon_nn_stats *stats)
{
    if (!s || !out_best || !out_row_ptr || (cols_cap && !out_cols)) return ISOCON_E_ARG;
    const uint32_t n = s->dev.n;
    HostClock clk0;
    if (getenv("ISOCON_DEBUG")) { (void)hipDeviceSynchronize(); clk0.lap("sync at entry"); }
    struct Total { std::chrono::steady_clock::time_point t = std::chrono::steady_clock::now();
                   ~Total() { if (getenv("ISOCON_DEBUG")) fprintf(stderr, "[isocon] %-28s %8.2f ms\n", "isocon_nn_graph total", std::chrono::duration<double, std::milli>(std::chrono::steady_clock::now() - t).count()); } } total;
    NNContext C;
    int rc = nn_setup(C, s, is_converged, is_target, depth, nullptr);
    if (rc) return rc;
    clk0.lap("setup");
    if (getenv("ISOCON_DEBUG")) { (void)hipDeviceSynchronize(); clk0.lap("sync after setup"); }
    C.keep_dev = n >= 1024 && !variant("nn_host_finalize");
    if ((rc = nn_phase_a(C, QMap{0u, n, 1u, 0u}, true, true, true))) return rc;
    HostClock clk;
    C.keep_dev = false;
    if (C.dev_hit_count) {
        bool wide = false;
        for (uint32_t q = 0; q < n && !wide; ++q) wide = C.qflag[q] && C.best[q] == NN_INF && s->lens[q] > 63;
        if (wide && (rc = C.pull_dev_hits())) return rc;
    }
    if ((rc = nn_phase_b(C, QMap{0u, n, 1u, 0u}))) return rc;
    clk.lap("phaseB");
    if (C.dev_hit_count) {
        if (C.hits.empty()) {
            C.stats.kernel_ms = C.tm.total; C.stats.narrow_kernel_ms = C.tm.marked_total;
            if (stats) *stats = C.stats;
            rc = nn_finalize_device_core(&s->pool, n, C.d_best.as<int32_t>(), C.best.data(), C.dev_hits, C.dev_hit_count, out_best, out_row_ptr, out_cols, cols_cap, n_cols_needed);
            clk.lap("finalize (device hits)");
            if (rc != ISOCON_E_UNSUPPORTED && rc != ISOCON_E_HIP) return rc;
        }
        if ((rc = C.pull_dev_hits())) return rc;
    }
    C.stats.kernel_ms = C.tm.total; C.stats.narrow_kernel_ms = C.tm.marked_total;
    if (stats) *stats = C.stats;
    struct Lap { HostClock &c; ~Lap() { c.lap("finalize"); } } lap{clk};
    if (C.hits.size() / 3 >= 4096 && n >= 1024 && !variant("nn_host_finalize")) {
        rc = nn_finalize_device(s, n, C.best.data(), C.hits.data(), C.hits.size() / 3, out_best, out_row_ptr, out_cols, cols_cap, n_cols_needed);
        if (rc != ISOCON_E_UNSUPPORTED && rc != ISOCON_E_HIP) return rc;
    }
    return nn_finalize_impl(n, C.best.data(), C.hits.data(), C.hits.size() / 3, out_best, out_row_ptr, out_cols, cols_cap, n_cols_needed);
}

extern "C" int isocon_qgram_bound_matrix(isocon_store *s, uint32_t q_begin, uint32_t q_end, uint32_t q_stride, uint32_t q_block, uint64_t depth,
                                         uint64_t *out_row_ptr, uint8_t *out_bounds, uint64_t bounds_cap, uint64_t *n_bounds_needed)
{
    if (!s || !out_row_ptr || !qmap_args_ok(q_stride, q_block) || (bounds_cap && !out_bounds)) return ISOCON_E_ARG;
    if (s->n_exc) { g_last_error = "q-gram bounds are defined on the 2-bit planes: the set holds more than four distinct symbols"; return ISOCON_E_ALPHABET; }
    const uint32_t n = s->dev.n;
    if (q_end > n) q_end = n;
    NNContext C;
    int rc = nn_setup(C, s, nullptr, nullptr, depth, nullptr);
    if (rc) return rc;
    NNParams P = C.params(63);
    s->pool.bound_tag.valid = false;
    const QMap Q = qmap_of(q_begin, q_end, q_stride, q_block);
    const uint32_t nq = Q.count();
    if ((rc = C.build_bounds(Q, 63, P))) return rc;
    ISO_HIP_CHECK(hipDeviceSynchronize());
    s->pool.bound_tag.valid = false;
    uint64_t total = 0;
    if (P.lb == nullptr) {
        for (uint32_t r = 0; r <= nq; ++r) out_row_ptr[r] = 0;
        if (n_bounds_needed) *n_bounds_needed = 0;
        bool any = false;
        for (uint32_t r = 0; r < C.lb_len_host.size(); ++r) any = any || C.lb_len_host[r] != 0;
        if (any) { g_last_error = "bound matrix not built (memory)"; return ISOCON_E_UNSUPPORTED; }
        return ISOCON_OK;
    }
    for (uint32_t r = 0; r < nq; ++r) { out_row_ptr[r] = total; total += C.lb_len_host[r]; }
    out_row_ptr[nq] = total;
    if (n_bounds_needed) *n_bounds_needed = total;
    if (total > bounds_cap) return ISOCON_E_CAPACITY;
    std::vector<uint8_t> raw((size_t)C.lb_total);
    ISO_HIP_CHECK(copy_d2h(raw.data(), P.lb, (size_t)C.lb_total));
    for (uint32_t r = 0; r < nq; ++r)
        if (C.lb_len_host[r]) memcpy(out_bounds + out_row_ptr[r], raw.data() + C.lb_off_host[r], C.lb_len_host[r]);
    if (C.d_lbt.p != nullptr) {
        std::vector<unsigned long long> offT(n);
        std::vector<uint32_t> sloT(n), lenT(n);
        ISO_HIP_CHECK(copy_d2h(offT.data(), C.d_offT.p, (size_t)n * 8));
        ISO_HIP_CHECK(copy_d2h(sloT.data(), C.d_sloT.p, (size_t)n * 4));
        ISO_HIP_CHECK(copy_d2h(lenT.data(), C.d_lenT.p, (size_t)n * 4));
        unsigned long long endT = 0, cells = 0;
        for (uint32_t p = 0; p < n; ++p) if (lenT[p]) endT = std::max(endT, offT[p] + lenT[p]);
        std::vector<uint8_t> rawT((size_t)endT + 1);
        if (endT) ISO_HIP_CHECK(copy_d2h(rawT.data(), C.d_lbt.p, (size_t)endT));
        for (uint32_t p = 0; p < n; ++p)
            for (uint32_t i = 0; i < lenT[p]; ++i) {
                const uint32_t r = sloT[p] + i;
                const uint64_t q = Q.entry(r);
                if (r >= nq || q >= p || p - q - 1 >= C.lb_len_host[r] || rawT[offT[p] + i] != raw[C.lb_off_host[r] + (p - q - 1)]) {
                    g_last_error = "transposed bound matrix differs from the matrix at entry " + std::to_string(p) + ", slot " + std::to_string(r);
                    return ISOCON_E_HIP;
                }
                ++cells;
            }
        if (cells != total) { g_last_error = "transposed bound matrix holds " + std::to_string(cells) + " cells, the matrix " + std::to_string(total); return ISOCON_E_HIP; }
    }
    return ISOCON_OK;
}
```

### isocon_amd/csrc/nn_lists.inc

```

namespace {

int NNContext::plan_lists(const QMap &Q, uint32_t nq, const NNParams &PR, ListPlan &L)
{
    L = ListPlan();
    if (PR.lb == nullptr || nq == 0 || variant("nn_no_list") || st->pool.slots[SLOT_NN_LBT].p == nullptr || st->maxlen >= 16384) return ISOCON_OK;
    unsigned long long pairs_cap = std::min<unsigned long long>(lb_total, std::max<unsigned long long>(1ull << 22, lb_total / 8));
    if (const char *e = variant_value("nn_list_cap")) pairs_cap = std::max<unsigned long long>(1, strtoull(e, nullptr, 10));
    const bool filter = !variant("nn_no_block_filter") && ensure_text2();
    uint32_t list_min = NN_LIST_MIN;
    if (const char *e = variant_value("nn_list_min")) list_min = (uint32_t)std::max(1, atoi(e));
    const uint32_t build_min = filter ? std::min<uint32_t>(list_min, NNF_LIST_MIN) : list_min;
    const unsigned long long cap_in = pairs_cap / build_min + 1, cap_out = filter ? pairs_cap / list_min + 1 : cap_in;
    size_t free_b = 0, total_b = 0;
    if (hipMemGetInfo(&free_b, &total_b) != hipSuccess || pairs_cap * 12 > free_b / 2 + st->pool.slots[SLOT_NN_LIST].cap * 3) return ISOCON_OK;
    DevBuf *bufs[] = {&d_ltot, &d_lchunks, &d_list, &d_lpa, &d_lpb, &d_lmeta, &d_ltasks};
    const int slots[] = {SLOT_NN_LTOT, SLOT_NN_LCHUNKS, SLOT_NN_LIST, SLOT_NN_LPA, SLOT_NN_LPB, SLOT_NN_LDEST, SLOT_NN_LTASKS};
    for (int i = 0; i < 7; ++i) { bufs[i]->pool = &st->pool; bufs[i]->slot = slots[i]; }
    const bool second = filter && !variant("nn_filter_one_pass");
    const unsigned long long tasks_cap = second ? 2 * cap_in + pairs_cap / 64 + 1 : 0;
    if (second && d_ltasks.alloc((size_t)tasks_cap * sizeof(NNFTask))) return ISOCON_OK;
    const size_t n_records = (size_t)(filter ? 2 * cap_in : 0) + 4 * (size_t)cap_out;
    if (d_lmeta.alloc((size_t)n * 4) || d_ltot.alloc(sizeof(NNPlanTotals)) || d_lchunks.alloc(n_records * sizeof(NNChunk)) || d_list.alloc((size_t)pairs_cap * 4) ||
        d_lpa.alloc((size_t)pairs_cap * 4) || d_lpb.alloc((size_t)pairs_cap * 4))
        return ISOCON_OK;
    NNChunk *built = d_lchunks.as<NNChunk>();
    L.a = built + (filter ? 2 * cap_in : 0);
    L.b = L.a + cap_out;
    L.sorted_a = L.b + cap_out;
    L.sorted_b = L.sorted_a + cap_out;
    ISO_HIP_CHECK(hipMemsetAsync(d_ltot.p, 0, sizeof(NNPlanTotals), 0));
    NNBoundRows B;
    B.lb = PR.lb; B.row_off = PR.lb_row; B.row_len = static_cast<const uint32_t *>(st->pool.slots[SLOT_NN_LBLEN].p);
    B.lbT = static_cast<const uint8_t *>(st->pool.slots[SLOT_NN_LBT].p);
    B.offT = static_cast<const unsigned long long *>(st->pool.slots[SLOT_NN_LBT_OFF].p);
    B.sloT = static_cast<const uint32_t *>(st->pool.slots[SLOT_NN_LBT_SLO].p);
    B.lenT = static_cast<const uint32_t *>(st->pool.slots[SLOT_NN_LBT_LEN].p);
    B.score = static_cast<const uint32_t *>(st->pool.slots[SLOT_NN_SCORE].p);
    tm.start();
    int32_t class_mode = 0;
    if (const char *e = variant_value("nn_narrow")) class_mode = atoi(e) > 0 ? 1 : -1;
    hipLaunchKernelGGL(k_nn_entry_meta, dim3((n + 255) / 256), dim3(256), 0, 0, st->dev, PR, B.score, d_lmeta.as<uint32_t>(), d_ltot.as<NNPlanTotals>());
    ISO_HIP_CHECK(hipGetLastError());
    hipLaunchKernelGGL(k_nn_survivors, dim3((n + NN_SURV_WAVES - 1) / NN_SURV_WAVES), dim3(64 * NN_SURV_WAVES), 0, 0, st->dev, PR, B, d_lmeta.as<uint32_t>(), Q, nq, d_list.as<uint32_t>(), pairs_cap,
                       filter ? built : L.a, cap_in, d_lpa.as<uint32_t>(), d_lpb.as<uint32_t>(), pairs_cap, d_ltot.as<NNPlanTotals>(), build_min, class_mode);
    ISO_HIP_CHECK(hipGetLastError());
    if (filter) {
        tm.mark();
        hipLaunchKernelGGL(k_nn_block_filter, dim3(NNF_GRID), dim3(256), 0, 0, d_text2.as<uint32_t>(), text2_stride, st->dev.lens, d_lmeta.as<uint32_t>(), PR.kcap, d_list.as<uint32_t>(),
                           built, cap_in, L.a, cap_out, d_lpa.as<uint32_t>(), d_lpb.as<uint32_t>(), pairs_cap, d_ltot.as<NNPlanTotals>(), list_min,
                           second ? d_ltasks.as<NNFTask>() : (NNFTask *)nullptr, tasks_cap);
        ISO_HIP_CHECK(hipGetLastError());
        if (second) {
            hipLaunchKernelGGL(k_nn_block_filter2, dim3(NNF_GRID2), dim3(256), 0, 0, d_text2.as<uint32_t>(), text2_stride, st->dev.lens, d_lmeta.as<uint32_t>(), PR.kcap,
                               d_list.as<uint32_t>(), d_ltasks.as<NNFTask>(), tasks_cap, d_lpa.as<uint32_t>(), d_lpb.as<uint32_t>(), pairs_cap, d_ltot.as<NNPlanTotals>());
            ISO_HIP_CHECK(hipGetLastError());
        }
    }
    NNPlanTotals tot;
    ISO_HIP_CHECK(hipMemcpy(&tot, d_ltot.p, sizeof(tot), hipMemcpyDeviceToHost));
    const float before = tm.marked_total;
    stats.list_kernel_ms += tm.stop();
    stats.filter_kernel_ms += tm.marked_total - before;
    tm.marked_total = before;
    if (tot.overflow) return ISOCON_OK;
    stats.pairs_prefiltered += tot.n_filtered;
    stats.pairs_block_rejected += tot.f_rejected + tot.f_rejected2;
    L.listed = true;
    L.n_chunks = filter ? tot.f_chunks : tot.n_chunks;
    L.n_chunks_narrow = filter ? tot.f_chunks_narrow : tot.n_chunks_narrow;
    L.n_small = tot.n_small;
    stats.pairs_wide_to_lanes += tot.n_wide_pairs;
    unsigned long long table_chunks = NNF_TABLE_CHUNKS;
    if (const char *e = variant_value("nn_table_chunks")) table_chunks = strtoull(e, nullptr, 10);
    if (filter && L.n_chunks + L.n_chunks_narrow > 0 && L.n_chunks + L.n_chunks_narrow < table_chunks) {
        if (tot.n_small + tot.f_listed > pairs_cap) return ISOCON_OK;
        L.conv_a = L.n_chunks; L.conv_b = L.n_chunks_narrow; L.conv_pairs = tot.f_listed;
        L.n_chunks = L.n_chunks_narrow = 0;
        return ISOCON_OK;
    }
    stats.pairs_narrow += filter ? tot.f_narrow_listed : tot.n_narrow_listed;
    return ISOCON_OK;
}

}
```

### isocon_amd/csrc/nn_main.inc

```

namespace {

int nn_phase_a_planes(NNContext &C, const QMap &Q, bool allow_regroup = false,
                      bool do_seed = true, bool do_main = true, bool seeded_before = false)
{
    const uint32_t n = C.n;
    const uint32_t q_begin = Q.begin, q_end = Q.end;
    if (q_begin >= q_end) return ISOCON_OK;
    const std::vector<int32_t> best0 = C.best;
    HostClock clk;
    for (;;) {
        int rc;
        if ((rc = C.upload_best()) || (rc = C.reset_counters())) return rc;
        clk.lap("phaseA: upload/reset");
        float ms = 0.f;
        std::vector<uint32_t> perm_used;
        std::vector<int32_t> seed_got;
        bool seed_collected = false;
        bool no_markers = false;
        bool seeds_clean = !do_seed;
        const bool two_set_lists = C.two_set && do_main && !variant("nn_tiles") && !variant("nn_no_qgram") &&
                                   n < (1u << 30) &&
                                   (size_t)std::count(C.tflag.begin(), C.tflag.end(), (uint8_t)1) > 512 &&
                                   ((size_t)4 * ((C.st->maxlen + 192 + 31) & ~31) + 160) * 4 + 16 * NN_RING * 8 + 16 <= (size_t)160 * 1024;
        if (!C.two_set || two_set_lists) {
            const uint32_t nq = Q.count();
            const bool refill_main = !variant("nn_tiles") &&
                                     ((size_t)4 * ((C.st->maxlen + 192 + 31) & ~31) + 160) * 4 + 16 * NN_RING * 8 + 16 <= (size_t)160 * 1024;
            const bool bounds_wanted = refill_main && !variant("nn_no_qgram");
            NNParams PR = C.params(63);
            bool bound_seeded = false, bounds_built = false;
            if (do_seed) {
                if (bounds_wanted && !variant("nn_old_seed")) {
                    if ((rc = C.build_bounds(Q, 63, PR, true))) return rc;
                    bounds_built = true;
                    clk.lap("phaseA: q-gram bounds");
                    if (C.seeds_ready) {
                        if ((rc = C.run_bound_seeds(Q))) return rc;
                        bound_seeded = true;
                        seeds_clean = true;
                        clk.lap("phaseA: seed pairs");
                    }
                }
                if (!bound_seeded) {
                    C.tm.start();
                    hipLaunchKernelGGL(k_nn_scan_up<1>, dim3((nq + 3) / 4), dim3(256), 0, 0, C.st->dev, C.params(63), Q, 0, 1, 1);
                    ISO_HIP_CHECK(hipGetLastError());
                    C.stats.seed_kernel_ms += C.tm.stop();
                    clk.lap("phaseA: seed kernel");
                }
            }
            std::vector<uint32_t> perm;
            DevStore S = C.st->dev;
            DevBuf d_planes2(&C.st->pool, SLOT_NN_PLANES2), d_perm(&C.st->pool, SLOT_NN_PERM), d_il(&C.st->pool, SLOT_NN_IL2);
            if (allow_regroup && !refill_main && do_seed && do_main && q_begin == 0 && q_end == n && Q.stride == 1 && Q.block_log2 == 0 && C.depth >= n && n > 128) {
                uint64_t needed0 = 0;
                std::vector<int32_t> seed_hits;
                rc = C.collect(seed_hits, &needed0);
                if (rc == ISOCON_OK) {
                    if ((rc = C.download_best())) return rc;
                    seed_got.swap(seed_hits);
                    std::vector<uint32_t> parent(n);
                    std::iota(parent.begin(), parent.end(), 0u);
                    auto find = [&](uint32_t x) { while (parent[x] != x) { parent[x] = parent[parent[x]]; x = parent[x]; } return x; };
                    for (size_t i = 0; i + 2 < seed_got.size(); i += 3) {
                        if (seed_got[i + 2] < 0) continue;
                        const uint32_t a = find((uint32_t)seed_got[i]), b = find((uint32_t)seed_got[i + 1]);
                        if (a != b) parent[a < b ? b : a] = a < b ? a : b;
                    }
                    perm.resize(n);
                    std::iota(perm.begin(), perm.end(), 0u);
                    std::vector<uint32_t> root(n);
                    for (uint32_t i = 0; i < n; ++i) root[i] = find(i);
                    const std::vector<int32_t> &lens = C.st->lens;
                    std::sort(perm.begin(), perm.end(), [&](uint32_t x, uint32_t y) {
                        if (lens[x] != lens[y]) return lens[x] < lens[y];
                        if (root[x] != root[y]) return root[x] < root[y];
                        if (C.best[x] != C.best[y]) return C.best[x] < C.best[y];
                        return x < y;
                    });
                    if (getenv("ISOCON_DEBUG")) {
                        std::vector<uint8_t> seen(n, 0);
                        bool okp = true;
                        for (uint32_t i = 0; i < n; ++i) { if (seen[perm[i]]) okp = false; seen[perm[i]] = 1; }
                        size_t ncomp = 0, moved = 0;
                        for (uint32_t i = 0; i < n; ++i) { ncomp += root[i] == i; moved += perm[i] != i; }
                        bool lens_ok = true;
                        for (uint32_t i = 0; i < n; ++i) lens_ok = lens_ok && lens[perm[i]] == lens[i];
                        fprintf(stderr, "[isocon] regroup: n=%u components=%zu moved=%zu perm_valid=%d lens_preserved=%d seed_hits=%zu\n",
                                n, ncomp, moved, (int)okp, (int)lens_ok, seed_got.size() / 3);
                    }
                    bool identity = true;
                    for (uint32_t i = 0; i < n && identity; ++i) identity = perm[i] == i;
                    if (identity) perm.clear();
                    else {
                        const size_t pbytes = (size_t)n * C.st->dev.nchunks * 16;
                        if ((rc = d_planes2.alloc(pbytes)) || (rc = d_perm.alloc((size_t)n * 4))) return rc;
                        ISO_HIP_CHECK(copy_h2d(d_perm.p, perm.data(), (size_t)n * 4));
                        C.tm.start();
                        hipLaunchKernelGGL(k_permute_planes, dim3(2048), dim3(256), 0, 0, reinterpret_cast<const ulonglong2 *>(C.st->dev.planes),
                                           d_planes2.as<ulonglong2>(), d_perm.as<uint32_t>(), n, C.st->dev.nchunks);
                        ISO_HIP_CHECK(hipGetLastError());
                        C.tm.stop();
                        S.planes = d_planes2.as<uint64_t>();
                        std::vector<int32_t> b2(n);
                        std::vector<uint8_t> q2(n), t2(n);
                        for (uint32_t i = 0; i < n; ++i) { b2[i] = C.best[perm[i]]; q2[i] = C.dev_excluded(perm[i]) ? 0 : C.qflag[perm[i]]; t2[i] = C.dev_excluded(perm[i]) ? 0 : C.tflag[perm[i]]; }
                        ISO_HIP_CHECK(copy_h2d(C.d_best.p, b2.data(), (size_t)n * 4));
                        ISO_HIP_CHECK(copy_h2d(C.d_qf.p, q2.data(), n));
                        ISO_HIP_CHECK(copy_h2d(C.d_tf.p, t2.data(), n));
                    }
                    if ((rc = C.reset_counters())) return rc;
                    seed_collected = true;
                    clk.lap("phaseA: regroup (host+permute)");
                } else if (rc != ISOCON_E_CAPACITY) return rc;
            }
            if (do_main) {
                const size_t lds = (size_t)(C.st->maxlen + 192) * 16;
                const int32_t first_tile = (perm.empty() && ((do_seed && !bound_seeded) || (seeded_before && !bounds_wanted))) ? 1 : 0;
                C.tm.start();
                const bool tiles_kernel = variant("nn_tiles");
                const size_t lds_r = ((size_t)4 * ((C.st->maxlen + 192 + 31) & ~31) + 160) * 4;
                const size_t ring8 = 8 * NN_RING * 8 + 16, ring16 = 16 * NN_RING * 8 + 16, cu_lds = 160 * 1024;
                if (n >= (1u << 30)) { g_last_error = "store too large for the packed neighbour queue"; return ISOCON_E_ARG; }
                bool refill = !tiles_kernel && lds_r + ring16 <= cu_lds && perm.empty();
                if (refill) refill = C.ensure_text();
                const uint32_t text_stride = C.text_stride;
                DevBuf &d_il_text = C.d_text;
                if (!refill && lds <= 160 * 1024) {
                    const size_t total = (size_t)n * C.st->dev.nchunks;
                    if ((rc = d_il.alloc(total * 16))) return rc;
                    hipLaunchKernelGGL(k_interleave_planes, dim3(2048), dim3(256), 0, 0, reinterpret_cast<const ulonglong2 *>(S.planes), d_il.as<ulonglong2>(), total);
                    S.il = d_il.as<uint64_t>();
                }
                if (refill && bounds_wanted && !bounds_built) {
                    ms += C.tm.stop();
                    if ((rc = C.build_bounds(Q, 63, PR))) return rc;
                    clk.lap("phaseA: q-gram bounds");
                    C.tm.start();
                }
                if (!refill) { PR.lb = nullptr; PR.lb_row = nullptr; PR.slot_order = nullptr; }
                const char *wv = variant_value("nn_waves");
                const bool four = wv ? atoi(wv) == 4 : PR.lb != nullptr;
                NNContext::ListPlan LP;
                if (refill && PR.lb != nullptr) {
                    ms += C.tm.stop();
                    if ((rc = C.plan_lists(Q, nq, PR, LP))) return rc;
                    clk.lap("phaseA: survivor lists");
                    C.tm.start();
                }
                const bool listed = LP.listed;
                const unsigned long long n_chunks = LP.n_chunks, n_chunks_narrow = LP.n_chunks_narrow, n_small = LP.n_small + LP.conv_pairs;
                no_markers = listed && seeds_clean;
                if (listed) {
                    NNParams PL = PR;
                    PL.list = C.d_list.as<uint32_t>();
                    PL.slot_order = nullptr;
                    const char *lw = variant_value("nn_list_waves");
                    const int lw64 = lw ? atoi(lw) : 4, lw32 = lw ? atoi(lw) : 8;
                    if (n_chunks) {
                        NNChunk *sorted = LP.sorted_a;
                        hipLaunchKernelGGL(k_nn_sort_chunks, dim3(1), dim3(1024), 0, 0, LP.a, (uint32_t)n_chunks, sorted);
                        ISO_HIP_CHECK(hipGetLastError());
                        PL.chunks = sorted;
                        if (const char *pad = variant_value("nn_lds_pad")) {
                            const size_t lds_p = lds_r + (size_t)atoi(pad);
                            ISO_HIP_CHECK(hipFuncSetAttribute((const void *)k_nn_scan_refill<8, 1>, hipFuncAttributeMaxDynamicSharedMemorySize, (int)lds_p));
                            hipLaunchKernelGGL((k_nn_scan_refill<8, 1>), dim3((unsigned)n_chunks), dim3(512), lds_p, 0, S, PL, d_il_text.as<uint32_t>(), text_stride, Q, 0);
                        } else if (lw64 == 4 && 3 * (lds_r + ring8) <= cu_lds) {
                            hipLaunchKernelGGL((k_nn_scan_refill<4, 1>), dim3((unsigned)n_chunks), dim3(256), lds_r, 0, S, PL, d_il_text.as<uint32_t>(), text_stride, Q, 0);
                        } else if (3 * (lds_r + ring8) <= cu_lds) {
                            hipLaunchKernelGGL((k_nn_scan_refill<8, 1>), dim3((unsigned)n_chunks), dim3(512), lds_r, 0, S, PL, d_il_text.as<uint32_t>(), text_stride, Q, 0);
                        } else {
                            ISO_HIP_CHECK(hipFuncSetAttribute((const void *)k_nn_scan_refill<16, 1>, hipFuncAttributeMaxDynamicSharedMemorySize, (int)lds_r));
                            hipLaunchKernelGGL((k_nn_scan_refill<16, 1>), dim3((unsigned)n_chunks), dim3(1024), lds_r, 0, S, PL, d_il_text.as<uint32_t>(), text_stride, Q, 0);
                        }
                        ISO_HIP_CHECK(hipGetLastError());
                    }
                    if (n_chunks_narrow) {
                        C.tm.mark();
                        NNChunk *sorted = LP.sorted_b;
                        hipLaunchKernelGGL(k_nn_sort_chunks, dim3(1), dim3(1024), 0, 0, LP.b, (uint32_t)n_chunks_narrow, sorted);
                        ISO_HIP_CHECK(hipGetLastError());
                        PL.chunks = sorted;
                        PL.stats = C.d_stats.as<unsigned long long>() + (NN_COUNTER_SLOTS * 4 + 1);
                        const size_t lds_h = ((size_t)4 * ((C.st->maxlen + 96 + 31) & ~31) + 96) * 4;
                        if (lw32 == 4 && 3 * (lds_h + ring8) <= cu_lds) {
                            hipLaunchKernelGGL((k_nn_scan_refill<4, 1, true>), dim3((unsigned)n_chunks_narrow), dim3(256), lds_h, 0, S, PL, d_il_text.as<uint32_t>(), text_stride, Q, 0);
                        } else if (3 * (lds_h + ring8) <= cu_lds) {
                            hipLaunchKernelGGL((k_nn_scan_refill<8, 1, true>), dim3((unsigned)n_chunks_narrow), dim3(512), lds_h, 0, S, PL, d_il_text.as<uint32_t>(), text_stride, Q, 0);
                        } else {
                            ISO_HIP_CHECK(hipFuncSetAttribute((const void *)k_nn_scan_refill<16, 1, true>, hipFuncAttributeMaxDynamicSharedMemorySize, (int)lds_h));
                            hipLaunchKernelGGL((k_nn_scan_refill<16, 1, true>), dim3((unsigned)n_chunks_narrow), dim3(1024), lds_h, 0, S, PL, d_il_text.as<uint32_t>(), text_stride, Q, 0);
                        }
                        ISO_HIP_CHECK(hipGetLastError());
                        PL.stats = C.d_stats.as<unsigned long long>();
                    }
                    if (n_small) {
                        ms += C.tm.stop();
                        C.tm.start();
                        const unsigned long long pairs_cap = C.st->pool.slots[SLOT_NN_LPA].cap / 4;
                        if (LP.conv_a) hipLaunchKernelGGL(k_nn_chunks_to_pairs, dim3((unsigned)LP.conv_a), dim3(256), 0, 0, LP.a, C.d_list.as<uint32_t>(), C.d_lpa.as<uint32_t>(), C.d_lpb.as<uint32_t>(), pairs_cap, C.d_ltot.as<NNPlanTotals>());
                        if (LP.conv_b) hipLaunchKernelGGL(k_nn_chunks_to_pairs, dim3((unsigned)LP.conv_b), dim3(256), 0, 0, LP.b, C.d_list.as<uint32_t>(), C.d_lpa.as<uint32_t>(), C.d_lpb.as<uint32_t>(), pairs_cap, C.d_ltot.as<NNPlanTotals>());
                        hipLaunchKernelGGL(k_ed_lanes<true>, dim3((unsigned)((n_small + 255) / 256)), dim3(256), 0, 0, C.st->dev, C.params(63), C.d_lpa.as<uint32_t>(), C.d_lpb.as<uint32_t>(),
                                           (const int32_t *)nullptr, (uint64_t)n_small, (int32_t *)nullptr);
                        ISO_HIP_CHECK(hipGetLastError());
                        C.stats.lanes_kernel_ms += C.tm.stop();
                        C.stats.pairs_evaluated += n_small;
                        C.stats.pairs_lanes += n_small;
                        C.tm.start();
                    }
                } else if (refill && four && 3 * (lds_r + ring8) <= cu_lds) {
                    hipLaunchKernelGGL((k_nn_scan_refill<4, 1>), dim3(nq), dim3(256), lds_r, 0, S, PR, d_il_text.as<uint32_t>(), text_stride, Q, first_tile);
                } else if (refill && 3 * (lds_r + ring8) <= cu_lds) {
                    hipLaunchKernelGGL((k_nn_scan_refill<8, 1>), dim3(nq), dim3(512), lds_r, 0, S, PR, d_il_text.as<uint32_t>(), text_stride, Q, first_tile);
                } else if (refill) {
                    ISO_HIP_CHECK(hipFuncSetAttribute((const void *)k_nn_scan_refill<16, 1>, hipFuncAttributeMaxDynamicSharedMemorySize, (int)lds_r));
                    hipLaunchKernelGGL((k_nn_scan_refill<16, 1>), dim3(nq), dim3(1024), lds_r, 0, S, PR, d_il_text.as<uint32_t>(), text_stride, Q, first_tile);
                } else if (lds <= 53 * 1024) {
                    hipLaunchKernelGGL(k_nn_scan_lds<8>, dim3(nq), dim3(512), lds, 0, S, C.params(63), Q, first_tile, 0x7fffffff);
                } else if (lds <= 160 * 1024) {
                    ISO_HIP_CHECK(hipFuncSetAttribute((const void *)k_nn_scan_lds<16>, hipFuncAttributeMaxDynamicSharedMemorySize, (int)lds));
                    hipLaunchKernelGGL(k_nn_scan_lds<16>, dim3(nq), dim3(1024), lds, 0, S, C.params(63), Q, first_tile, 0x7fffffff);
                } else {
                    hipLaunchKernelGGL(k_nn_scan_up<1>, dim3(nq), dim3(256), 0, 0, S, C.params(63), Q, first_tile, 0x7fffffff, 4);
                }
                ISO_HIP_CHECK(hipGetLastError());
                ms += C.tm.stop();
                C.stats.scan_launches += 1;
            }
            if (!do_main) no_markers = do_seed && seeds_clean;
            perm_used.swap(perm);
            clk.lap("phaseA: main kernel");
        } else if (do_main && !variant("nn_tiles") && n < (1u << 30) &&
                   (size_t)std::count(C.tflag.begin(), C.tflag.end(), (uint8_t)1) > 512 &&
                   ((size_t)4 * ((C.st->maxlen + 192 + 31) & ~31) + 160) * 4 + 16 * NN_RING * 8 + 16 <= (size_t)160 * 1024 && C.ensure_text()) {
            const uint32_t nq = Q.count();
            const size_t lds_r = ((size_t)4 * ((C.st->maxlen + 192 + 31) & ~31) + 160) * 4, ring8 = 8 * NN_RING * 8 + 16;
            NNParams PR = C.params(63);
            if ((rc = C.build_bounds(Q, 63, PR))) return rc;
            C.tm.start();
            if (3 * (lds_r + ring8) <= (size_t)160 * 1024) {
                hipLaunchKernelGGL((k_nn_scan_refill<8, 1>), dim3(nq), dim3(512), lds_r, 0, C.st->dev, PR, C.d_text.as<uint32_t>(), C.text_stride,
                                   Q, 0);
            } else {
                ISO_HIP_CHECK(hipFuncSetAttribute((const void *)k_nn_scan_refill<16, 1>, hipFuncAttributeMaxDynamicSharedMemorySize, (int)lds_r));
                hipLaunchKernelGGL((k_nn_scan_refill<16, 1>), dim3(nq), dim3(1024), lds_r, 0, C.st->dev, PR, C.d_text.as<uint32_t>(), C.text_stride,
                                   Q, 0);
            }
            ISO_HIP_CHECK(hipGetLastError());
            ms += C.tm.stop();
            C.stats.scan_launches += 1;
        } else {
            std::vector<uint32_t> ts, ids, lanes;
            for (uint32_t c = 0; c < n && do_main; ++c) {
                if (!C.tflag[c] || C.dev_excluded(c)) continue;
                uint32_t lo, hi;
                length_window(C.st->lens, c, 63, lo, hi);
                lo = std::max(lo, q_begin);
                hi = std::min(hi, q_end);
                lanes.clear();
                for (uint32_t p = lo; p < hi; ++p)
                    if (C.qflag[p] && !C.dev_excluded(p) && Q.owns(p)) lanes.push_back(p);
                push_tiles(ts, ids, c, lanes);
            }
            if ((rc = run_nn_tiles(1, C, ts, ids, &ms))) return rc;
            C.stats.scan_launches += 1;
        }
        C.stats.scan_kernel_ms += ms;
        uint64_t needed = 0;
        std::vector<int32_t> got;
        const bool dev_ok = C.keep_dev && no_markers && perm_used.empty() && !seed_collected && C.hits.empty();
        rc = C.collect(got, &needed, perm_used.empty(), dev_ok);
        if (rc == ISOCON_E_CAPACITY) {
            C.hits_cap = needed + needed / 2 + 1024;
            if ((rc = C.d_hits.alloc(C.hits_cap * 12))) return rc;
            if (perm_used.empty()) {
                if ((rc = C.download_best())) return rc;
            } else {
                C.best = best0;
                if ((rc = C.upload_flags())) return rc;
            }
            continue;
        }
        if (rc) return rc;
        if ((rc = C.download_best())) return rc;
        if (dev_ok) { clk.lap("phaseA: hits stay on the device"); return ISOCON_OK; }
        if (!perm_used.empty()) {
            std::vector<int32_t> b(n);
            for (uint32_t i = 0; i < n; ++i) b[perm_used[i]] = C.best[i];
            std::copy(b.begin(), b.end(), C.best.begin());
            for (size_t i = 0; i + 2 < got.size(); i += 3) { got[i] = (int32_t)perm_used[got[i]]; got[i + 1] = (int32_t)perm_used[got[i + 1]]; }
            if ((rc = C.upload_flags())) return rc;
        }
        if (seed_collected) got.insert(got.end(), seed_got.begin(), seed_got.end());
        clk.lap("phaseA: collect+unpermute");
        std::vector<uint32_t> ra, rb;
        bool any_marker = false;
        for (size_t i = 2; i < got.size() && !any_marker; i += 3) any_marker = got[i] == -2;
        if (!any_marker) C.hits.insert(C.hits.end(), got.begin(), got.end());
        else {
            C.hits.reserve(C.hits.size() + got.size());
            for (size_t i = 0; i + 2 < got.size(); i += 3) {
                if (got[i + 2] == -2) { ra.push_back((uint32_t)got[i]); rb.push_back((uint32_t)got[i + 1]); }
                else C.hits.insert(C.hits.end(), got.begin() + i, got.begin() + i + 3);
            }
        }
        if (!ra.empty()) {
            std::vector<int32_t> kk(ra.size(), 63), dd(ra.size(), -1);
            float ems = 0.f;
            if ((rc = ed_pairs_impl(C.st, ra.data(), rb.data(), kk.data(), ra.size(), dd.data(), &ems, nullptr, C.image_pass))) return rc;
            C.tm.total += ems;
            for (size_t i = 0; i < ra.size(); ++i)
                if (dd[i] >= 0) C.apply(ra[i], rb[i], dd[i]);
        }
        clk.lap("phaseA: markers");
        return ISOCON_OK;
    }
}


}
```

Before: 72.09 billion alignments/s.

## Defer event timing, stage uploads via pinned arena, cache free-memory query

Replaces the synchronous event timer with deferred event records that are resolved at the next sync point. Host-to-device uploads go through a pinned staging arena with async copies, and memsets are made async. hipMemGetInfo is cached per context, and the device-resident collect path is merged into a single batched async readback with one stream sync. Text allocation is postponed until after list planning shows it is needed. The aim is to remove the host stalls and implicit syncs between kernels during NN-graph construction. The risks are extra bookkeeping, a stale free-memory estimate, and pinned memory that grows over time.

New measurement: 73.09 billion alignments/s (median of 3 runs). No clear change (+1.4%).

```diff
diff --git a/isocon_amd/csrc/isocon_hip.hip b/isocon_amd/csrc/isocon_hip.hip
--- a/isocon_amd/csrc/isocon_hip.hip
+++ b/isocon_amd/csrc/isocon_hip.hip
@@ -239,25 +239,95 @@
     return ISOCON_OK;
 }
 
+struct PinnedArena {
+    struct Chunk { char *p; size_t cap, used; };
+    std::vector<Chunk> chunks;
+    void *take(size_t bytes)
+    {
+        bytes = (bytes + 255) & ~(size_t)255;
+        if (chunks.empty() || chunks.back().cap - chunks.back().used < bytes) {
+            void *p = nullptr;
+            const size_t cap = std::max(bytes, (size_t)4 << 20);
+            if (hipHostMalloc(&p, cap, hipHostMallocDefault) != hipSuccess) { (void)hipGetLastError(); return nullptr; }
+            chunks.push_back(Chunk{static_cast<char *>(p), cap, 0});
+        }
+        Chunk &c = chunks.back();
+        void *r = c.p + c.used;
+        c.used += bytes;
+        return r;
+    }
+    void reset()
+    {
+        if (chunks.size() > 1) {
+            size_t all = 0;
+            for (Chunk &c : chunks) { all += c.cap; (void)hipHostFree(c.p); }
+            chunks.clear();
+            void *p = nullptr;
+            if (hipHostMalloc(&p, all, hipHostMallocDefault) == hipSuccess) chunks.push_back(Chunk{static_cast<char *>(p), all, 0});
+            else (void)hipGetLastError();
+        }
+        for (Chunk &c : chunks) c.used = 0;
+    }
+    void release() { for (Chunk &c : chunks) (void)hipHostFree(c.p); chunks.clear(); }
+};
+static PinnedArena g_arena;
+
+static hipError_t copy_h2d_queued(void *ddst, const void *src, size_t bytes)
+{
+    void *h = g_arena.take(bytes);
+    if (!h) return copy_h2d(ddst, src, bytes);
+    memcpy(h, src, bytes);
+    return hipMemcpyAsync(ddst, h, bytes, hipMemcpyHostToDevice, 0);
+}
+
 struct EventTimer {
-    hipEvent_t e0 = nullptr, e1 = nullptr, em = nullptr;
     float total = 0.f;
     float marked_total = 0.f;
     bool marked = false;
-    bool ok = false;
-    EventTimer() { ok = hipEventCreate(&e0) == hipSuccess && hipEventCreate(&e1) == hipSuccess && hipEventCreate(&em) == hipSuccess; }
-    ~EventTimer() { if (e0) (void)hipEventDestroy(e0); if (e1) (void)hipEventDestroy(e1); if (em) (void)hipEventDestroy(em); }
-    void start() { if (ok) (void)hipEventRecord(e0, 0); marked = false; }
-    void mark() { if (ok) { (void)hipEventRecord(em, 0); marked = true; } }
-    float stop()
+    bool deferred = false;
+    struct Pending { hipEvent_t e0, em, e1; float *dst, *marked_dst; };
+    std::vector<Pending> pending;
+    std::vector<hipEvent_t> mine, spare;
+    hipEvent_t e0 = nullptr, em = nullptr;
+    EventTimer() {}
+    EventTimer(const EventTimer &) = delete;
+    EventTimer &operator=(const EventTimer &) = delete;
+    ~EventTimer() { for (hipEvent_t e : mine) (void)hipEventDestroy(e); }
+    hipEvent_t event()
     {
-        float ms = 0.f;
-        if (ok) {
-            (void)hipEventRecord(e1, 0); (void)hipEventSynchronize(e1); (void)hipEventElapsedTime(&ms, e0, e1);
-            if (marked) { float part = 0.f; (void)hipEventElapsedTime(&part, em, e1); marked_total += part; marked = false; }
-        }
-        total += ms;
-        return ms;
+        hipEvent_t e = nullptr;
+        if (!spare.empty()) { e = spare.back(); spare.pop_back(); return e; }
+        if (hipEventCreate(&e) != hipSuccess) { (void)hipGetLastError(); return nullptr; }
+        mine.push_back(e);
+        return e;
+    }
+    void start() { e0 = event(); em = nullptr; marked = false; if (e0) (void)hipEventRecord(e0, 0); }
+    void mark() { em = event(); if (em) { (void)hipEventRecord(em, 0); marked = true; } }
+    void stop(float *dst, float *marked_dst = nullptr)
+    {
+        hipEvent_t e1 = e0 ? event() : nullptr;
+        if (e1) {
+            (void)hipEventRecord(e1, 0);
+            pending.push_back(Pending{e0, marked ? em : nullptr, e1, dst, marked_dst});
+        }
+        e0 = em = nullptr;
+        marked = false;
+        if (!deferred && e1) { (void)hipEventSynchronize(e1); resolve(); }
+    }
+    float stop() { float ms = 0.f; const bool d = deferred; deferred = false; stop(&ms); deferred = d; return ms; }
+    void resolve()
+    {
+        for (const Pending &p : pending) {
+            float ms = 0.f, part = 0.f;
+            if (hipEventElapsedTime(&ms, p.e0, p.e1) != hipSuccess) { (void)hipGetLastError(); ms = 0.f; }
+            if (p.em && hipEventElapsedTime(&part, p.em, p.e1) != hipSuccess) { (void)hipGetLastError(); part = 0.f; }
+            total += ms;
+            if (p.dst) *p.dst += ms;
+            if (p.em) { if (p.marked_dst) *p.marked_dst += part; else marked_total += part; spare.push_back(p.em); }
+            spare.push_back(p.e0);
+            spare.push_back(p.e1);
+        }
+        pending.clear();
     }
 };
 
@@ -326,7 +396,7 @@
     return n;
 }
 
-void isocon_release_scratch(void) { g_scratch.release(); g_stage.release(); }
+void isocon_release_scratch(void) { g_scratch.release(); g_stage.release(); g_arena.release(); }
 
 int isocon_init(int device_ordinal)
 {
diff --git a/isocon_amd/csrc/nn_bounds.inc b/isocon_amd/csrc/nn_bounds.inc
--- a/isocon_amd/csrc/nn_bounds.inc
+++ b/isocon_amd/csrc/nn_bounds.inc
@@ -25,15 +25,15 @@
     d_qprof.slot = SLOT_NN_QPROF; d_qsum.slot = SLOT_NN_QSUM;
     HostClock bclk;
     {
-        size_t free_b = 0, total_b = 0;
-        if (hipMemGetInfo(&free_b, &total_b) != hipSuccess || prof_bytes > free_b / 2 + st->pool.slots[SLOT_NN_QPROF].cap) return ISOCON_OK;
+        size_t free_b = 0;
+        if (!mem_free(free_b) || prof_bytes > free_b / 2 + st->pool.slots[SLOT_NN_QPROF].cap) return ISOCON_OK;
         if (d_qprof.alloc(prof_bytes) || d_qsum.alloc((size_t)n * 4)) return ISOCON_OK;
     }
     bclk.lap("bounds: memory check + profile buffers");
     tm.start();
     hipLaunchKernelGGL(k_qgram_profile4, dim3((n + QP_SEQS - 1) / QP_SEQS), dim3(256), 0, 0, st->dev, d_qprof.as<uint8_t>(), d_qsum.as<uint32_t>(), n_pad);
     ISO_HIP_CHECK(hipGetLastError());
-    struct StopTimer { NNContext &c; bool armed = true; ~StopTimer() { if (armed) c.stats.bound_kernel_ms += c.tm.stop(); } } stop_timer{*this};
+    struct StopTimer { NNContext &c; bool armed = true; ~StopTimer() { if (armed) c.tm.stop(&c.stats.bound_kernel_ms); } } stop_timer{*this};
     std::vector<unsigned long long> &off = lb_off_host;
     std::vector<uint32_t> &rlen = lb_len_host;
     off.assign(nq, 0);
@@ -62,9 +62,9 @@
     bclk.lap("bounds: profile launch + rows (host)");
     const unsigned long long totalT = sum_rlen + 30ull * n;
     bclk.lap("bounds: transposed rows (host)");
-    size_t free_b = 0, total_b = 0;
+    size_t free_b = 0;
     const size_t need = (size_t)total + (size_t)totalT + prof_bytes + (size_t)n * 24 + (size_t)nq * 12;
-    if (hipMemGetInfo(&free_b, &total_b) != hipSuccess || need > free_b / 2 + st->pool.slots[SLOT_NN_LB].cap + st->pool.slots[SLOT_NN_QPROF].cap) return ISOCON_OK;
+    if (!mem_free(free_b) || need > free_b / 2 + st->pool.slots[SLOT_NN_LB].cap + st->pool.slots[SLOT_NN_QPROF].cap) return ISOCON_OK;
     bclk.lap("bounds: memory check 2");
     std::vector<uint2> tiles;
     for (uint32_t g = 0; g * 4 < nrb; ++g) {
@@ -101,9 +101,9 @@
     d_chunks.pool = &st->pool;
     d_chunks.slot = SLOT_NN_LBCHUNKS;
     if (d_chunks.alloc(tiles.size() * sizeof(uint2))) return ISOCON_OK;
-    ISO_HIP_CHECK(copy_h2d(d_chunks.p, tiles.data(), tiles.size() * sizeof(uint2)));
-    ISO_HIP_CHECK(copy_h2d(d_lbrow.p, off.data(), (size_t)nq * 8));
-    ISO_HIP_CHECK(copy_h2d(d_lblen.p, rlen.data(), (size_t)nq * 4));
+    ISO_HIP_CHECK(copy_h2d_queued(d_chunks.p, tiles.data(), tiles.size() * sizeof(uint2)));
+    ISO_HIP_CHECK(copy_h2d_queued(d_lbrow.p, off.data(), (size_t)nq * 8));
+    ISO_HIP_CHECK(copy_h2d_queued(d_lblen.p, rlen.data(), (size_t)nq * 4));
     hipLaunchKernelGGL(k_lbt_rows, dim3((n + 255) / 256), dim3(256), 0, 0, Q, nq, d_lblen.as<uint32_t>(), n, d_sloT.as<uint32_t>(), d_lenT.as<uint32_t>(), d_padT.as<uint32_t>());
     if ((rc = device_exscan<0, unsigned long long>(&st->pool, d_padT.as<uint32_t>(), n, d_offT.as<unsigned long long>()))) return ISOCON_OK;
     hipLaunchKernelGGL(k_lbt_offsets, dim3((n + 255) / 256), dim3(256), 0, 0, n, d_sloT.as<uint32_t>(), d_offT.as<unsigned long long>());
@@ -116,7 +116,7 @@
         d_order.pool = &st->pool;
         d_order.slot = SLOT_NN_SLOTORDER;
         if (d_order.alloc((size_t)nq * 4)) return ISOCON_OK;
-        ISO_HIP_CHECK(copy_h2d(d_order.p, order.data(), (size_t)nq * 4));
+        ISO_HIP_CHECK(copy_h2d_queued(d_order.p, order.data(), (size_t)nq * 4));
     }
     unsigned long long *rowmin = nullptr, *colmin = nullptr;
     if (want_seeds) {
@@ -142,13 +142,8 @@
                        d_lbt.as<uint8_t>(), d_score.as<uint32_t>());
     ISO_HIP_CHECK(hipGetLastError());
     stop_timer.armed = false;
-    {
-        const float before = tm.marked_total;
-        stats.bound_kernel_ms += tm.stop();
-        stats.mm_kernel_ms += tm.marked_total - before;
-        tm.marked_total = before;
-    }
-    bclk.lap("bounds: k_qgram_mm (wait)");
+    tm.stop(&stats.bound_kernel_ms, &stats.mm_kernel_ms);
+    bclk.lap("bounds: k_qgram_mm (queued)");
 #ifdef ISOCON_QM_TIMELINE
     {
         const size_t nt = std::min<size_t>(tiles.size(), 16384);
@@ -204,7 +199,7 @@
     hipLaunchKernelGGL(k_ed_lanes<true>, dim3((unsigned)((np + 255) / 256)), dim3(256), 0, 0, st->dev, params(63), d_seed_a.as<uint32_t>(), d_seed_b.as<uint32_t>(),
                        (const int32_t *)nullptr, np, (int32_t *)nullptr);
     ISO_HIP_CHECK(hipGetLastError());
-    stats.seed_kernel_ms += tm.stop();
+    tm.stop(&stats.seed_kernel_ms);
     return ISOCON_OK;
 }
 
diff --git a/isocon_amd/csrc/nn_context.inc b/isocon_amd/csrc/nn_context.inc
--- a/isocon_amd/csrc/nn_context.inc
+++ b/isocon_amd/csrc/nn_context.inc
@@ -36,10 +36,29 @@
     isocon_nn_stats stats;
     EventTimer tm;
 
-    bool ensure_text()
+    bool mem_known = false;
+    size_t mem_free_b = 0;
+    bool mem_free(size_t &free_b)
+    {
+        if (!mem_known) {
+            size_t total_b = 0;
+            if (hipMemGetInfo(&mem_free_b, &total_b) != hipSuccess) { (void)hipGetLastError(); return false; }
+            mem_known = true;
+        }
+        free_b = mem_free_b;
+        return true;
+    }
+    bool text_feasible()
     {
         if (text_ready) return true;
         text_stride = (uint32_t)NN_TEXT_PAD_FRONT + (uint32_t)((st->maxlen + 7) / 8) + (uint32_t)NN_TEXT_PAD_BACK;
+        size_t free_b = 0;
+        return mem_free(free_b) && (size_t)n * text_stride * 4 <= free_b / 2;
+    }
+    bool ensure_text()
+    {
+        if (text_ready) return true;
+        if (!text_feasible()) return false;
         size_t free_b = 0, total_b = 0;
         if (hipMemGetInfo(&free_b, &total_b) != hipSuccess || (size_t)n * text_stride * 4 > free_b / 2) return false;
         d_text.pool = &st->pool;
@@ -57,8 +76,8 @@
     {
         if (text2_ready) return true;
         text2_stride = nnf_text2_stride(st->maxlen);
-        size_t free_b = 0, total_b = 0;
-        if (hipMemGetInfo(&free_b, &total_b) != hipSuccess || (size_t)n * text2_stride * 4 > free_b / 2 + st->pool.slots[SLOT_NN_TEXT2].cap) return false;
+        size_t free_b = 0;
+        if (!mem_free(free_b) || (size_t)n * text2_stride * 4 > free_b / 2 + st->pool.slots[SLOT_NN_TEXT2].cap) return false;
         d_text2.pool = &st->pool;
         d_text2.slot = SLOT_NN_TEXT2;
         if (d_text2.alloc((size_t)std::max<uint32_t>(n, 1) * text2_stride * 4) != ISOCON_OK) return false;
@@ -112,25 +131,25 @@
         return P;
     }
 
-    int upload_best() { ISO_HIP_CHECK(copy_h2d(d_best.p, best.data(), (size_t)n * 4)); return ISOCON_OK; }
+    int upload_best(bool queued = false)
+    {
+        ISO_HIP_CHECK(queued ? copy_h2d_queued(d_best.p, best.data(), (size_t)n * 4) : copy_h2d(d_best.p, best.data(), (size_t)n * 4));
+        return ISOCON_OK;
+    }
     int download_best() { ISO_HIP_CHECK(copy_d2h(best.data(), d_best.p, (size_t)n * 4)); return ISOCON_OK; }
     int reset_counters()
     {
-        ISO_HIP_CHECK(hipMemset(d_hit_count.p, 0, 8));
-        ISO_HIP_CHECK(hipMemset(d_stats.p, 0, 2 * (NN_COUNTER_SLOTS * 4 + 1) * 8));
+        ISO_HIP_CHECK(hipMemsetAsync(d_hit_count.p, 0, 8, 0));
+        ISO_HIP_CHECK(hipMemsetAsync(d_stats.p, 0, 2 * (NN_COUNTER_SLOTS * 4 + 1) * 8, 0));
         return ISOCON_OK;
     }
     bool keep_dev = false;
     const int32_t *dev_hits = nullptr;
     uint64_t dev_hit_count = 0;
-    int collect(std::vector<int32_t> &out, uint64_t *needed, bool filter = false, bool to_device = false)
-    {
-        unsigned long long cnt = 0;
-        ISO_HIP_CHECK(hipMemcpy(&cnt, d_hit_count.p, 8, hipMemcpyDeviceToHost));
-        unsigned long long sc2[2][NN_COUNTER_SLOTS * 4 + 1];
-        ISO_HIP_CHECK(hipMemcpy(sc2, d_stats.p, sizeof(sc2), hipMemcpyDeviceToHost));
+    void add_counters(const unsigned long long *sc2)
+    {
         for (int blk = 0; blk < 2; ++blk) {
-            const unsigned long long *sc = sc2[blk];
+            const unsigned long long *sc = sc2 + blk * (NN_COUNTER_SLOTS * 4 + 1);
             stats.pairs_prefiltered += sc[NN_COUNTER_SLOTS * 4];
             for (int i = 0; i < NN_COUNTER_SLOTS; ++i) {
                 stats.pairs_evaluated += sc[i * 4 + 0];
@@ -140,21 +159,68 @@
                 if (blk == 1) stats.narrow_columns += sc[i * 4 + 1];
             }
         }
+    }
+    bool csr_follows = false;
+    int filter_hits_dev(unsigned long long &cnt, const void *&src)
+    {
+        DevBuf d_h2(&st->pool, SLOT_NN_HITS2), d_c2(&st->pool, SLOT_NN_HITCOUNT2);
+        int rc;
+        if ((rc = d_h2.alloc((size_t)cnt * 12)) || (rc = d_c2.alloc(8))) return rc;
+        ISO_HIP_CHECK(hipMemsetAsync(d_c2.p, 0, 8, 0));
+        const unsigned blocks = (unsigned)std::min<unsigned long long>((cnt + 255) / 256, 4096);
+        hipLaunchKernelGGL(k_filter_hits, dim3(blocks), dim3(256), 0, 0, d_hits.as<int32_t>(), cnt, d_best.as<int32_t>(), d_h2.as<int32_t>(),
+                           d_c2.as<unsigned long long>());
+        ISO_HIP_CHECK(hipGetLastError());
+        ISO_HIP_CHECK(hipMemcpy(&cnt, d_c2.p, 8, hipMemcpyDeviceToHost));
+        src = d_h2.p;
+        return ISOCON_OK;
+    }
+    int collect_dev(uint64_t *needed)
+    {
+        const size_t sc_bytes = 2 * (NN_COUNTER_SLOTS * 4 + 1) * 8, sc_room = (sc_bytes + 255) & ~(size_t)255;
+        char *h = static_cast<char *>(g_arena.take(256 + sc_room + (size_t)n * 4));
+        if (!h || dev_hit_count != 0) {
+            std::vector<int32_t> none;
+            const int rc = collect(none, needed, true, true);
+            tm.resolve();
+            if (rc) return rc;
+            return download_best();
+        }
+        ISO_HIP_CHECK(hipMemcpyAsync(h, d_hit_count.p, 8, hipMemcpyDeviceToHost, 0));
+        ISO_HIP_CHECK(hipMemcpyAsync(h + 256, d_stats.p, sc_bytes, hipMemcpyDeviceToHost, 0));
+        ISO_HIP_CHECK(hipMemcpyAsync(h + 256 + sc_room, d_best.p, (size_t)n * 4, hipMemcpyDeviceToHost, 0));
+        ISO_HIP_CHECK(hipStreamSynchronize(0));
+        tm.resolve();
+        unsigned long long cnt = 0;
+        memcpy(&cnt, h, 8);
+        add_counters(reinterpret_cast<const unsigned long long *>(h + 256));
+        memcpy(best.data(), h + 256 + sc_room, (size_t)n * 4);
+        if (needed) *needed = cnt;
+        if (cnt > hits_cap) return ISOCON_E_CAPACITY;
+        stats.hits += cnt;
+        const void *src = d_hits.p;
+        if (!csr_follows && cnt > 4096) {
+            const int rc = filter_hits_dev(cnt, src);
+            if (rc) return rc;
+        }
+        dev_hits = static_cast<const int32_t *>(src);
+        dev_hit_count = cnt;
+        return ISOCON_OK;
+    }
+    int collect(std::vector<int32_t> &out, uint64_t *needed, bool filter = false, bool to_device = false)
+    {
+        unsigned long long cnt = 0;
+        ISO_HIP_CHECK(hipMemcpy(&cnt, d_hit_count.p, 8, hipMemcpyDeviceToHost));
+        unsigned long long sc2[2 * (NN_COUNTER_SLOTS * 4 + 1)];
+        ISO_HIP_CHECK(hipMemcpy(sc2, d_stats.p, sizeof(sc2), hipMemcpyDeviceToHost));
+        add_counters(sc2);
         if (needed) *needed = cnt;
         if (cnt > hits_cap) return ISOCON_E_CAPACITY;
         stats.hits += cnt;
         const void *src = d_hits.p;
         if (filter && cnt > 4096 && dev_hit_count == 0) {
-            DevBuf d_h2(&st->pool, SLOT_NN_HITS2), d_c2(&st->pool, SLOT_NN_HITCOUNT2);
-            int rc;
-            if ((rc = d_h2.alloc((size_t)cnt * 12)) || (rc = d_c2.alloc(8))) return rc;
-            ISO_HIP_CHECK(hipMemset(d_c2.p, 0, 8));
-            const unsigned blocks = (unsigned)std::min<unsigned long long>((cnt + 255) / 256, 4096);
-            hipLaunchKernelGGL(k_filter_hits, dim3(blocks), dim3(256), 0, 0, d_hits.as<int32_t>(), cnt, d_best.as<int32_t>(), d_h2.as<int32_t>(),
-                               d_c2.as<unsigned long long>());
-            ISO_HIP_CHECK(hipGetLastError());
-            ISO_HIP_CHECK(hipMemcpy(&cnt, d_c2.p, 8, hipMemcpyDeviceToHost));
-            src = d_h2.p;
+            const int rc = filter_hits_dev(cnt, src);
+            if (rc) return rc;
         }
         if (to_device) {
             dev_hits = static_cast<const int32_t *>(src);
@@ -187,8 +253,8 @@
     {
         if (!n) return ISOCON_OK;
         if (!st->n_exc || !mask_exc) {
-            ISO_HIP_CHECK(copy_h2d(d_qf.p, qflag.data(), n));
-            ISO_HIP_CHECK(copy_h2d(d_tf.p, tflag.data(), n));
+            ISO_HIP_CHECK(copy_h2d_queued(d_qf.p, qflag.data(), n));
+            ISO_HIP_CHECK(copy_h2d_queued(d_tf.p, tflag.data(), n));
             return ISOCON_OK;
         }
         std::vector<uint8_t> q2(qflag), t2(tflag);
@@ -262,6 +328,8 @@
     C.d_best.slot = SLOT_NN_BEST; C.d_qf.slot = SLOT_NN_QF; C.d_tf.slot = SLOT_NN_TF; C.d_hits.slot = SLOT_NN_HITS;
     C.d_hit_count.slot = SLOT_NN_HITCOUNT; C.d_stats.slot = SLOT_NN_STATS;
     const uint32_t n = C.n;
+    ISO_HIP_CHECK(hipStreamSynchronize(0));
+    g_arena.reset();
     for (uint32_t i = 1; i < n; ++i)
         if (s->lens[i] < s->lens[i - 1]) { g_last_error = "nearest-neighbour entry points need a length-sorted store"; return ISOCON_E_ARG; }
     C.two_set = is_target != nullptr;
diff --git a/isocon_amd/csrc/nn_entry.inc b/isocon_amd/csrc/nn_entry.inc
--- a/isocon_amd/csrc/nn_entry.inc
+++ b/isocon_amd/csrc/nn_entry.inc
@@ -36,10 +36,13 @@
     hipLaunchKernelGGL(k_fin_gather, dim3(nb_), dim3(256), 0, 0, n, d_start.as<unsigned long long>(), d_nb.as<uint32_t>(), d_rowptr.as<unsigned long long>(), d_cols.as<uint32_t>());
     ISO_HIP_CHECK(hipGetLastError());
     uint32_t flag = 0;
-    ISO_HIP_CHECK(hipMemcpy(&flag, d_flag.p, 4, hipMemcpyDeviceToHost));
-    if (flag) return ISOCON_E_UNSUPPORTED;
+    uint32_t *h_flag = static_cast<uint32_t *>(g_arena.take(4));
+    if (h_flag) ISO_HIP_CHECK(hipMemcpyAsync(h_flag, d_flag.p, 4, hipMemcpyDeviceToHost, 0));
+    else ISO_HIP_CHECK(hipMemcpy(&flag, d_flag.p, 4, hipMemcpyDeviceToHost));
     static_assert(sizeof(unsigned long long) == sizeof(uint64_t), "row pointers travel as they are");
     ISO_HIP_CHECK(copy_d2h(out_row_ptr, d_rowptr.p, ((size_t)n + 1) * 8));
+    if (h_flag) { ISO_HIP_CHECK(hipStreamSynchronize(0)); flag = *h_flag; }
+    if (flag) return ISOCON_E_UNSUPPORTED;
     const uint64_t total = out_row_ptr[n];
     if (n_cols_needed) *n_cols_needed = total;
     if (total > cols_cap) return ISOCON_E_CAPACITY;
@@ -162,6 +165,7 @@
     if (!s || !out_row_ptr || (n_rows && !hits_dev) || (cols_cap && !out_cols)) return ISOCON_E_ARG;
     const uint32_t n = s->dev.n;
     if (n && (!best_dev || !out_best)) return ISOCON_E_ARG;
+    g_arena.reset();
     std::vector<int32_t> best(std::max<uint32_t>(n, 1));
     if (n) ISO_HIP_CHECK(copy_d2h(best.data(), best_dev, (size_t)n * 4));
     int rc = nn_finalize_device_core(&s->pool, n, best_dev, best.data(), hits_dev, n_rows, out_best, out_row_ptr, out_cols, cols_cap, n_cols_needed);
@@ -187,6 +191,7 @@
     clk0.lap("setup");
     if (getenv("ISOCON_DEBUG")) { (void)hipDeviceSynchronize(); clk0.lap("sync after setup"); }
     C.keep_dev = n >= 1024 && !variant("nn_host_finalize");
+    C.csr_follows = C.keep_dev;
     if ((rc = nn_phase_a(C, QMap{0u, n, 1u, 0u}, true, true, true))) return rc;
     HostClock clk;
     C.keep_dev = false;
diff --git a/isocon_amd/csrc/nn_lists.inc b/isocon_amd/csrc/nn_lists.inc
--- a/isocon_amd/csrc/nn_lists.inc
+++ b/isocon_amd/csrc/nn_lists.inc
@@ -12,8 +12,8 @@
     if (const char *e = variant_value("nn_list_min")) list_min = (uint32_t)std::max(1, atoi(e));
     const uint32_t build_min = filter ? std::min<uint32_t>(list_min, NNF_LIST_MIN) : list_min;
     const unsigned long long cap_in = pairs_cap / build_min + 1, cap_out = filter ? pairs_cap / list_min + 1 : cap_in;
-    size_t free_b = 0, total_b = 0;
-    if (hipMemGetInfo(&free_b, &total_b) != hipSuccess || pairs_cap * 12 > free_b / 2 + st->pool.slots[SLOT_NN_LIST].cap * 3) return ISOCON_OK;
+    size_t free_b = 0;
+    if (!mem_free(free_b) || pairs_cap * 12 > free_b / 2 + st->pool.slots[SLOT_NN_LIST].cap * 3) return ISOCON_OK;
     DevBuf *bufs[] = {&d_ltot, &d_lchunks, &d_list, &d_lpa, &d_lpb, &d_lmeta, &d_ltasks};
     const int slots[] = {SLOT_NN_LTOT, SLOT_NN_LCHUNKS, SLOT_NN_LIST, SLOT_NN_LPA, SLOT_NN_LPB, SLOT_NN_LDEST, SLOT_NN_LTASKS};
     for (int i = 0; i < 7; ++i) { bufs[i]->pool = &st->pool; bufs[i]->slot = slots[i]; }
@@ -57,12 +57,13 @@
             ISO_HIP_CHECK(hipGetLastError());
         }
     }
+    tm.stop(&stats.list_kernel_ms, &stats.filter_kernel_ms);
     NNPlanTotals tot;
-    ISO_HIP_CHECK(hipMemcpy(&tot, d_ltot.p, sizeof(tot), hipMemcpyDeviceToHost));
-    const float before = tm.marked_total;
-    stats.list_kernel_ms += tm.stop();
-    stats.filter_kernel_ms += tm.marked_total - before;
-    tm.marked_total = before;
+    if (void *h_tot = g_arena.take(sizeof(NNPlanTotals))) {
+        ISO_HIP_CHECK(hipMemcpyAsync(h_tot, d_ltot.p, sizeof(tot), hipMemcpyDeviceToHost, 0));
+        ISO_HIP_CHECK(hipStreamSynchronize(0));
+        memcpy(&tot, h_tot, sizeof(tot));
+    } else ISO_HIP_CHECK(hipMemcpy(&tot, d_ltot.p, sizeof(tot), hipMemcpyDeviceToHost));
     if (tot.overflow) return ISOCON_OK;
     stats.pairs_prefiltered += tot.n_filtered;
     stats.pairs_block_rejected += tot.f_rejected + tot.f_rejected2;
diff --git a/isocon_amd/csrc/nn_main.inc b/isocon_amd/csrc/nn_main.inc
--- a/isocon_amd/csrc/nn_main.inc
+++ b/isocon_amd/csrc/nn_main.inc
@@ -9,9 +9,14 @@
     if (q_begin >= q_end) return ISOCON_OK;
     const std::vector<int32_t> best0 = C.best;
     HostClock clk;
+    struct Deferred {
+        EventTimer &t;
+        explicit Deferred(EventTimer &tm) : t(tm) { t.deferred = true; }
+        ~Deferred() { t.deferred = false; if (!t.pending.empty()) { (void)hipStreamSynchronize(0); t.resolve(); } }
+    } deferred_times(C.tm);
     for (;;) {
         int rc;
-        if ((rc = C.upload_best()) || (rc = C.reset_counters())) return rc;
+        if ((rc = C.upload_best(true)) || (rc = C.reset_counters())) return rc;
         clk.lap("phaseA: upload/reset");
         float ms = 0.f;
         std::vector<uint32_t> perm_used;
@@ -46,7 +51,7 @@
                     C.tm.start();
                     hipLaunchKernelGGL(k_nn_scan_up<1>, dim3((nq + 3) / 4), dim3(256), 0, 0, C.st->dev, C.params(63), Q, 0, 1, 1);
                     ISO_HIP_CHECK(hipGetLastError());
-                    C.stats.seed_kernel_ms += C.tm.stop();
+                    C.tm.stop(&C.stats.seed_kernel_ms);
                     clk.lap("phaseA: seed kernel");
                 }
             }
@@ -124,33 +129,34 @@
                 const size_t ring8 = 8 * NN_RING * 8 + 16, ring16 = 16 * NN_RING * 8 + 16, cu_lds = 160 * 1024;
                 if (n >= (1u << 30)) { g_last_error = "store too large for the packed neighbour queue"; return ISOCON_E_ARG; }
                 bool refill = !tiles_kernel && lds_r + ring16 <= cu_lds && perm.empty();
-                if (refill) refill = C.ensure_text();
+                if (refill) refill = C.text_feasible();
                 const uint32_t text_stride = C.text_stride;
                 DevBuf &d_il_text = C.d_text;
+                if (refill && bounds_wanted && !bounds_built) {
+                    C.tm.stop(&C.stats.scan_kernel_ms);
+                    if ((rc = C.build_bounds(Q, 63, PR))) return rc;
+                    clk.lap("phaseA: q-gram bounds");
+                    C.tm.start();
+                }
+                const char *wv = variant_value("nn_waves");
+                const bool four = wv ? atoi(wv) == 4 : PR.lb != nullptr;
+                NNContext::ListPlan LP;
+                if (refill && PR.lb != nullptr) {
+                    C.tm.stop(&C.stats.scan_kernel_ms);
+                    if ((rc = C.plan_lists(Q, nq, PR, LP))) return rc;
+                    clk.lap("phaseA: survivor lists");
+                    C.tm.start();
+                }
+                bool listed = LP.listed;
+                const unsigned long long n_chunks = LP.n_chunks, n_chunks_narrow = LP.n_chunks_narrow, n_small = LP.n_small + LP.conv_pairs;
+                if (refill && (!listed || n_chunks || n_chunks_narrow) && !C.ensure_text()) { refill = false; listed = false; }
                 if (!refill && lds <= 160 * 1024) {
                     const size_t total = (size_t)n * C.st->dev.nchunks;
                     if ((rc = d_il.alloc(total * 16))) return rc;
                     hipLaunchKernelGGL(k_interleave_planes, dim3(2048), dim3(256), 0, 0, reinterpret_cast<const ulonglong2 *>(S.planes), d_il.as<ulonglong2>(), total);
                     S.il = d_il.as<uint64_t>();
                 }
-                if (refill && bounds_wanted && !bounds_built) {
-                    ms += C.tm.stop();
-                    if ((rc = C.build_bounds(Q, 63, PR))) return rc;
-                    clk.lap("phaseA: q-gram bounds");
-                    C.tm.start();
-                }
                 if (!refill) { PR.lb = nullptr; PR.lb_row = nullptr; PR.slot_order = nullptr; }
-                const char *wv = variant_value("nn_waves");
-                const bool four = wv ? atoi(wv) == 4 : PR.lb != nullptr;
-                NNContext::ListPlan LP;
-                if (refill && PR.lb != nullptr) {
-                    ms += C.tm.stop();
-                    if ((rc = C.plan_lists(Q, nq, PR, LP))) return rc;
-                    clk.lap("phaseA: survivor lists");
-                    C.tm.start();
-                }
-                const bool listed = LP.listed;
-                const unsigned long long n_chunks = LP.n_chunks, n_chunks_narrow = LP.n_chunks_narrow, n_small = LP.n_small + LP.conv_pairs;
                 no_markers = listed && seeds_clean;
                 if (listed) {
                     NNParams PL = PR;
@@ -197,7 +203,7 @@
                         PL.stats = C.d_stats.as<unsigned long long>();
                     }
                     if (n_small) {
-                        ms += C.tm.stop();
+                        C.tm.stop(&C.stats.scan_kernel_ms);
                         C.tm.start();
                         const unsigned long long pairs_cap = C.st->pool.slots[SLOT_NN_LPA].cap / 4;
                         if (LP.conv_a) hipLaunchKernelGGL(k_nn_chunks_to_pairs, dim3((unsigned)LP.conv_a), dim3(256), 0, 0, LP.a, C.d_list.as<uint32_t>(), C.d_lpa.as<uint32_t>(), C.d_lpb.as<uint32_t>(), pairs_cap, C.d_ltot.as<NNPlanTotals>());
@@ -205,7 +211,7 @@
                         hipLaunchKernelGGL(k_ed_lanes<true>, dim3((unsigned)((n_small + 255) / 256)), dim3(256), 0, 0, C.st->dev, C.params(63), C.d_lpa.as<uint32_t>(), C.d_lpb.as<uint32_t>(),
                                            (const int32_t *)nullptr, (uint64_t)n_small, (int32_t *)nullptr);
                         ISO_HIP_CHECK(hipGetLastError());
-                        C.stats.lanes_kernel_ms += C.tm.stop();
+                        C.tm.stop(&C.stats.lanes_kernel_ms);
                         C.stats.pairs_evaluated += n_small;
                         C.stats.pairs_lanes += n_small;
                         C.tm.start();
@@ -226,7 +232,7 @@
                     hipLaunchKernelGGL(k_nn_scan_up<1>, dim3(nq), dim3(256), 0, 0, S, C.params(63), Q, first_tile, 0x7fffffff, 4);
                 }
                 ISO_HIP_CHECK(hipGetLastError());
-                ms += C.tm.stop();
+                C.tm.stop(&C.stats.scan_kernel_ms);
                 C.stats.scan_launches += 1;
             }
             if (!do_main) no_markers = do_seed && seeds_clean;
@@ -249,7 +255,7 @@
                                    Q, 0);
             }
             ISO_HIP_CHECK(hipGetLastError());
-            ms += C.tm.stop();
+            C.tm.stop(&C.stats.scan_kernel_ms);
             C.stats.scan_launches += 1;
         } else {
             std::vector<uint32_t> ts, ids, lanes;
@@ -271,7 +277,9 @@
         uint64_t needed = 0;
         std::vector<int32_t> got;
         const bool dev_ok = C.keep_dev && no_markers && perm_used.empty() && !seed_collected && C.hits.empty();
-        rc = C.collect(got, &needed, perm_used.empty(), dev_ok);
+        rc = dev_ok ? C.collect_dev(&needed) : C.collect(got, &needed, perm_used.empty(), false);
+        C.tm.resolve();
+        if (dev_ok && rc == ISOCON_OK) { clk.lap("phaseA: hits stay on the device"); return ISOCON_OK; }
         if (rc == ISOCON_E_CAPACITY) {
             C.hits_cap = needed + needed / 2 + 1024;
             if ((rc = C.d_hits.alloc(C.hits_cap * 12))) return rc;
@@ -285,7 +293,6 @@
         }
         if (rc) return rc;
         if ((rc = C.download_best())) return rc;
-        if (dev_ok) { clk.lap("phaseA: hits stay on the device"); return ISOCON_OK; }
         if (!perm_used.empty()) {
             std::vector<int32_t> b(n);
             for (uint32_t i = 0; i < n; ++i) b[perm_used[i]] = C.best[i];
```
